# aosokin/os2d

Measured on AMD Instinct MI355X. Metric: query-image-pairs/s (1280-px input, ResNet50, N-class), higher is better.
Workload: dtype fftx3 (as fft; the per-bin complex GEMM on the fp16 MFMA with spectra split into fp16 hi+lo, 3 MFMAs per product, fp32 accumulate)

## Files before the change

### include/os2d_hip.h

```cpp
#ifndef OS2D_HIP_H
#define OS2D_HIP_H

#include <stddef.h>

#ifdef __cplusplus
extern "C" {
#endif

#define OS2D_ABI_VERSION 9

#define OS2D_PRECISION_F32 0
#define OS2D_PRECISION_F16X3 1
#define OS2D_PRECISION_F16X2 2

#define OS2D_PRECISION_FFT 3

#define OS2D_PRECISION_FFT32 5

#define OS2D_PRECISION_FFTX3 4

int os2d_abi_version(void);

const char* os2d_last_error(void);

size_t os2d_packed_conv_floats(int layer );
size_t os2d_packed_bias_floats(int layer );
int os2d_pack_conv(int layer, int P, const float* w, const float* b, const float* bn_weight, const float* bn_bias,
                   const float* bn_running_mean, const float* bn_running_var, float bn_eps, float* packed_w,
                   float* packed_b, void* stream);

int os2d_class_prepare(const float* src, int C, int h, int w, int normalize, float* q15, float* qp, void* stream);
size_t os2d_class_prepare_workspace_floats(int B, int C);
int os2d_class_prepare_batch(const float* const* srcs, const int* sizes, int B, int C, int normalize, float* q15,
                             float* qp, float* workspace, void* stream);

int os2d_head_workspace_bytes(int A, int B, int C, int H, int W, int P, size_t* bytes);
int os2d_head_workspace_bytes_ex(int A, int B, int C, int H, int W, int P, int precision, size_t* bytes);
int os2d_head_forward(const float* fm, const float* qp, const float* w1, const float* b1, const float* w2,
                      const float* b2, const float* w3, const float* b3, int A, int B, int C, int H, int W, int P,
                      int inverse, int stride, int rec_field, float* loc, float* cls, float* corners,
                      void* workspace, size_t workspace_bytes, void* stream);

size_t os2d_packed_conv_bytes(int layer, int precision);
int os2d_rnorm_exp(void);
int os2d_pack_conv_f16x3(int layer , int P, const float* w, const float* b, const float* bn_weight,
                         const float* bn_bias, const float* bn_running_mean, const float* bn_running_var, float bn_eps,
                         const int* weight_exp, const int* in_exp, const int* out_exp, void* packed_w, float* packed_b,
                         void* stream);

size_t os2d_class_split_bytes(int B, int C);
int os2d_class_split(const float* qp, void* qs, int B, int C, void* stream);

#define OS2D_STATUS_F16_RANGE 1
int os2d_head_forward_ex(const float* fm, const float* qp, const void* w1, const float* b1, const void* w2,
                         const float* b2, const void* w3, const float* b3, int A, int B, int C, int H, int W, int P,
                         int inverse, int stride, int rec_field, float* loc, float* cls, float* corners,
                         void* workspace, size_t workspace_bytes, void* stream, int precision, const void* qs,
                         void** stage_events, int* chunk_classes, int* status, const float* wspec, const float* twQ,
                         const float* twP);
int os2d_head_forward_ex2(const float* fm, const float* qp, const void* w1, const float* b1, const void* w2,
                          const float* b2, const void* w3, const float* b3, int A, int B, int C, int H, int W, int P,
                          int inverse, int stride, int rec_field, float* loc, float* cls, float* corners,
                          void* workspace, size_t workspace_bytes, void* stream, int precision, const void* qs,
                          void** stage_events, int* chunk_classes, int* status, const float* wspec, const float* twQ,
                          const float* twP, const void* wspec2);
void os2d_debug_set_dump(void* stream, int slot, void* dst, size_t bytes);
int os2d_prof_event_create(void** ev);
int os2d_prof_event_destroy(void* ev);
int os2d_prof_event_elapsed_ms(void* begin, void* end, float* ms);

int os2d_fm_sumsq(const float* fm, float* sumsq, int A, int C, int H, int W, void* stream);
size_t os2d_plane_floats(int H, int W);
int os2d_corr(const float* fm, const float* qp, const float* sumsq, float* corr, float* rnorm, int A, int B, int C,
              int H, int W, void* stream);
size_t os2d_corr_f16x3_workspace_bytes(int A, int C, int H, int W);
int os2d_corr_f16x3(const float* fm, const void* qs, float* corr, void* rshb, int A, int B, int C, int H, int W,
                    void* workspace, size_t workspace_bytes, void* stream);
size_t os2d_corr_f16x3_packed_workspace_bytes(int A, int B, int C, int H, int W);
int os2d_corr_f16x3_packed(const float* fm, const void* qs, float* corr, float* inv_norm, int A, int B, int C, int H, int W,
                           int form, void* workspace, size_t workspace_bytes, void* stream);
int os2d_corr_normalize(const float* corr, float* rnorm, int NB, int H, int W, void* stream);
int os2d_transform_conv(int layer, const float* in, const float* packed_w, const float* packed_b, float* out,
                        int NB, int P, int H, int W, void* stream);
size_t os2d_shb_bytes(int channels, int H, int W);
int os2d_corr_normalize_f16x3(const float* corr, void* rshb, int NB, int H, int W, void* stream);
int os2d_transform_conv_f16x3(int layer, const void* in, const void* packed_w, const float* packed_b, void* out, int NB,
                              int P, int H, int W, int terms, int* status, void* stream);
int os2d_alignment_grids(const float* params, int NB, int H, int W, int P, int inverse, float* theta, float* grids,
                         void* stream);
int os2d_sample_decode(const float* corr, const float* params, int NB, int H, int W, int P, int inverse, int stride,
                       int rec_field, float* loc, float* cls, float* corners, void* stream);

int os2d_decode_boxes(const float* loc, int NB, int H, int W, int stride, int rec_field, float img_w, float img_h,
                      float* boxes, void* stream);

int os2d_nms_workspace_bytes(int NC, int N, size_t* bytes);
int os2d_nms(const float* boxes, const int* counts, int NC, int N, float iou_threshold, unsigned char* keep,
             int* num_keep, void* workspace, size_t workspace_bytes, void* stream);

int os2d_detect_level_supported(int H, int W);
int os2d_detect_level(const float* loc, const float* cls, int B, int H, int W, int stride, int rec_field, float img_w,
                      float img_h, float scale_x, float scale_y, float score_threshold, float iou_threshold,
                      float* out_boxes, float* out_scores, int* out_index, int* out_count, void* stream);

#define OS2D_BOX_OP_SCALE 1
#define OS2D_BOX_OP_HFLIP 2
#define OS2D_BOX_OP_VFLIP 3
#define OS2D_BOX_OP_SHIFT 4
#define OS2D_BOX_MAX_OPS 6
#define OS2D_BOX_MAX_DEFAULT_OPS 12
int os2d_detect_level_ops(const float* loc, const float* cls, int B, int H, int W, int stride, int rec_field, float img_w,
                          float img_h, int op_count, const int* op_kinds, const float* op_args, float score_threshold,
                          float iou_threshold, float* out_boxes, float* out_scores, int* out_index, int* out_count,
                          void* stream);

size_t os2d_spectral_weight_bytes(int C, int Cout, int nbins);
int os2d_fft_sizes(int H, int W, int* P, int* Q, int* nbins);
int os2d_fft_tiles(int H, int W, int* tiles_y, int* tiles_x, int* tile_h, int* tile_w);
int os2d_fft_forward(const float* corr, const float* inv_norm, float* X, const float* twQ, const float* twP, int NB, int C,
                     int H, int W, void* stream);
int os2d_fft_inverse(const float* Y, const float* packed_b, void* out, const float* twQ, const float* twP, int NB, int Cout,
                     int H, int W, int* status, void* stream);
#define OS2D_SPECTRA_ROWS 0
#define OS2D_SPECTRA_QUADS 1
int os2d_fft_inverse_ex(const float* Y, const float* packed_b, void* out, const float* twQ, const float* twP, int NB, int Cout,
                        int H, int W, int* status, int layout, void* stream);
int os2d_spectral_gemm(const float* wspec, const float* X, float* Y, int NB, int C, int Cout, int nbins, void* stream);
size_t os2d_spectral_weight16_bytes(int C, int nbins);
int os2d_spectral_weights_build(const double* wfold, const double* twP64, const double* twQ64, int C, int Cout, int P, int Q,
                                int nbins, int split, void* out, void* workspace, void* stream);
float os2d_spectral_xscale(int H, int W);
int os2d_spectral_gemm_f16(const void* w16, const float* X, float* Y, int NB, int C, int Cout, int nbins, float xscale,
                           void* stream);

int os2d_dft_sizes(int H, int W, int* P, int* Q, int* nbins, int* tiles);
int os2d_dft_channel_stride(int C);
size_t os2d_dft_matrices_bytes(int P, int Q);
int os2d_dft_matrices_build(const double* twP64, const double* twQ64, int P, int Q, void* out, void* stream);
int os2d_dft_forward(const float* corr, const float* inv_norm, float* X, const void* matrices, int NB, int C, int H, int W,
                     void* stream);
int os2d_dft_inverse(const float* Y, const float* packed_b, void* out, const void* matrices, int NB, int Cout, int H, int W,
                     int* status, void* stream);
int os2d_dft_inverse_planes(const float* Y, const float* packed_b, float* out, const void* matrices, int NB, int Cout, int H, int W,
                            int* status, void* stream);
int os2d_spectral_weights_build_dft(const double* wfold, const double* twP64, const double* twQ64, int C, int Cout, int P, int Q,
                                    int nbins, void* out, void* workspace, void* stream);
int os2d_spectral_gemm_f16_quads(const void* w16, const float* X, float* Y, int NB, int C, int Cout, int nbins, float xscale,
                                 void* stream);
float os2d_dft_xscale(int H, int W);

#define OS2D_PYRAMID_MAX_LEVELS 16
int os2d_detect_pyramid_supported(int L, int N, int nms_max_batch);
int os2d_detect_pyramid_workspace_bytes(int B, int N, int passes, size_t* bytes);
int os2d_detect_pyramid(const float* const* loc, const float* const* cls, const float* const* corners, int B, int L,
                        const int* hw, int stride, int rec_field, const float* img_wh, const float* scale_xy,
                        float score_threshold, float iou_threshold, int nms_max_batch, int passes, float* out_boxes,
                        float* out_scores, int* out_index, float* out_default, float* out_corners, int* out_count,
                        int* unfinished, void* workspace, size_t workspace_bytes, void* stream);
int os2d_detect_pyramid_merged(const float* const* loc, const float* const* cls, const float* const* corners, int B, int L,
                               const int* hw, int stride, int rec_field, const float* img_wh, const float* scale_xy,
                               float score_threshold, float iou_threshold, int nms_max_batch, int passes, int G, int V,
                               const int* slot_rows, float* out_boxes, float* out_scores, int* out_index, float* out_default,
                               float* out_corners, int* out_count, int* unfinished, void* workspace, size_t workspace_bytes,
                               void* stream);

int os2d_detect_pyramid_ops(const float* const* loc, const float* const* cls, const float* const* corners, int B, int L,
                            const int* hw, int stride, int rec_field, const float* img_wh, const int* op_counts,
                            const int* op_kinds, const float* op_args, const int* default_op_counts,
                            const int* default_op_kinds, const float* default_op_args, float score_threshold, float iou_threshold,
                            int nms_max_batch, int passes, int G, int V, const int* slot_rows, float* out_boxes,
                            float* out_scores, int* out_index, float* out_default, float* out_corners, int* out_count,
                            int* unfinished, void* workspace, size_t workspace_bytes, void* stream);

#ifdef __cplusplus
}
#endif
#endif
```

### os2d_amd/_lib.py

```python
import ctypes

from . import build
from ._native import NativeLibrary, Os2dLibraryError, ptr, host_ptr, current_stream

ABI_VERSION = 9

_c_float_p = ctypes.c_void_p
_vp = ctypes.c_void_p
_i = ctypes.c_int
_f = ctypes.c_float
_sz = ctypes.c_size_t

SIGNATURES = {
    "os2d_abi_version": (_i, []),
    "os2d_last_error": (ctypes.c_char_p, []),
    "os2d_packed_conv_floats": (_sz, [_i]),
    "os2d_packed_bias_floats": (_sz, [_i]),
    "os2d_pack_conv": (_i, [_i, _i, _vp, _vp, _vp, _vp, _vp, _vp, _f, _vp, _vp, _vp]),
    "os2d_class_prepare": (_i, [_vp, _i, _i, _i, _i, _vp, _vp, _vp]),
    "os2d_head_workspace_bytes": (_i, [_i, _i, _i, _i, _i, _i, ctypes.POINTER(_sz)]),
    "os2d_head_forward": (_i, [_vp] * 8 + [_i] * 9 + [_vp, _vp, _vp, _vp, _sz, _vp]),
    "os2d_packed_conv_bytes": (_sz, [_i, _i]),
    "os2d_pack_conv_f16x3": (_i, [_i, _i, _vp, _vp, _vp, _vp, _vp, _vp, _f, _vp, _vp, _vp, _vp, _vp, _vp]),
    "os2d_rnorm_exp": (_i, []),
    "os2d_class_prepare_batch": (_i, [_vp, _vp, _i, _i, _i, _vp, _vp, _vp, _vp]),
    "os2d_class_prepare_workspace_floats": (_sz, [_i, _i]),
    "os2d_shb_bytes": (_sz, [_i, _i, _i]),
    "os2d_corr_normalize_f16x3": (_i, [_vp, _vp, _i, _i, _i, _vp]),
    "os2d_transform_conv_f16x3": (_i, [_i, _vp, _vp, _vp, _vp, _i, _i, _i, _i, _i, _vp, _vp]),
    "os2d_alignment_grids": (_i, [_vp, _i, _i, _i, _i, _i, _vp, _vp, _vp]),
    "os2d_spectral_weight_bytes": (_sz, [_i, _i, _i]),
    "os2d_spectral_gemm": (_i, [_vp, _vp, _vp, _i, _i, _i, _i, _vp]),
    "os2d_spectral_weight16_bytes": (_sz, [_i, _i]),
    "os2d_spectral_xscale": (_f, [_i, _i]),
    "os2d_spectral_weights_build": (_i, [_vp, _vp, _vp, _i, _i, _i, _i, _i, _i, _vp, _vp, _vp]),
    "os2d_spectral_gemm_f16": (_i, [_vp, _vp, _vp, _i, _i, _i, _i, _f, _vp]),
    "os2d_debug_set_dump": (None, [_vp, _i, _vp, _sz]),
    "os2d_fft_sizes": (_i, [_i, _i, ctypes.POINTER(_i), ctypes.POINTER(_i), ctypes.POINTER(_i)]),
    "os2d_fft_tiles": (_i, [_i, _i, ctypes.POINTER(_i), ctypes.POINTER(_i), ctypes.POINTER(_i), ctypes.POINTER(_i)]),
    "os2d_fft_forward": (_i, [_vp, _vp, _vp, _vp, _vp, _i, _i, _i, _i, _vp]),
    "os2d_fft_inverse": (_i, [_vp, _vp, _vp, _vp, _vp, _i, _i, _i, _i, _vp, _vp]),
    "os2d_fft_inverse_ex": (_i, [_vp, _vp, _vp, _vp, _vp, _i, _i, _i, _i, _vp, _i, _vp]),
    "os2d_dft_sizes": (_i, [_i, _i, ctypes.POINTER(_i), ctypes.POINTER(_i), ctypes.POINTER(_i), ctypes.POINTER(_i)]),
    "os2d_dft_channel_stride": (_i, [_i]),
    "os2d_dft_matrices_bytes": (_sz, [_i, _i]),
    "os2d_dft_matrices_build": (_i, [_vp, _vp, _i, _i, _vp, _vp]),
    "os2d_dft_forward": (_i, [_vp, _vp, _vp, _vp, _i, _i, _i, _i, _vp]),
    "os2d_dft_inverse": (_i, [_vp, _vp, _vp, _vp, _i, _i, _i, _i, _vp, _vp]),
    "os2d_spectral_weights_build_dft": (_i, [_vp, _vp, _vp, _i, _i, _i, _i, _i, _vp, _vp, _vp]),
    "os2d_spectral_gemm_f16_quads": (_i, [_vp, _vp, _vp, _i, _i, _i, _i, _f, _vp]),
    "os2d_dft_xscale": (_f, [_i, _i]),
    "os2d_class_split": (_i, [_vp, _vp, _i, _i, _vp]),
    "os2d_class_split_bytes": (_sz, [_i, _i]),
    "os2d_head_forward_ex": (_i, [_vp] * 8 + [_i] * 9 + [_vp, _vp, _vp, _vp, _sz, _vp, _i, _vp,
                                  ctypes.POINTER(_vp), ctypes.POINTER(_i), _vp, _vp, _vp, _vp]),
    "os2d_head_forward_ex2": (_i, [_vp] * 8 + [_i] * 9 + [_vp, _vp, _vp, _vp, _sz, _vp, _i, _vp,
                                   ctypes.POINTER(_vp), ctypes.POINTER(_i), _vp, _vp, _vp, _vp, _vp]),
    "os2d_dft_inverse_planes": (_i, [_vp, _vp, _vp, _vp, _i, _i, _i, _i, _vp, _vp]),
    "os2d_head_workspace_bytes_ex": (_i, [_i, _i, _i, _i, _i, _i, _i, ctypes.POINTER(_sz)]),
    "os2d_prof_event_create": (_i, [ctypes.POINTER(_vp)]),
    "os2d_prof_event_destroy": (_i, [_vp]),
    "os2d_prof_event_elapsed_ms": (_i, [_vp, _vp, ctypes.POINTER(_f)]),
    "os2d_fm_sumsq": (_i, [_vp, _vp, _i, _i, _i, _i, _vp]),
    "os2d_plane_floats": (_sz, [_i, _i]),
    "os2d_corr": (_i, [_vp, _vp, _vp, _vp, _vp, _i, _i, _i, _i, _i, _vp]),
    "os2d_corr_normalize": (_i, [_vp, _vp, _i, _i, _i, _vp]),
    "os2d_corr_f16x3_workspace_bytes": (_sz, [_i, _i, _i, _i]),
    "os2d_corr_f16x3": (_i, [_vp, _vp, _vp, _vp, _i, _i, _i, _i, _i, _vp, _sz, _vp]),
    "os2d_corr_f16x3_packed_workspace_bytes": (_sz, [_i, _i, _i, _i, _i]),
    "os2d_corr_f16x3_packed": (_i, [_vp, _vp, _vp, _vp, _i, _i, _i, _i, _i, _i, _vp, _sz, _vp]),
    "os2d_transform_conv": (_i, [_i, _vp, _vp, _vp, _vp, _i, _i, _i, _i, _vp]),
    "os2d_sample_decode": (_i, [_vp, _vp, _i, _i, _i, _i, _i, _i, _i, _vp, _vp, _vp, _vp]),
    "os2d_decode_boxes": (_i, [_vp, _i, _i, _i, _i, _i, _f, _f, _vp, _vp]),
    "os2d_nms_workspace_bytes": (_i, [_i, _i, ctypes.POINTER(_sz)]),
    "os2d_nms": (_i, [_vp, _vp, _i, _i, _f, _vp, _vp, _vp, _sz, _vp]),
    "os2d_detect_level_supported": (_i, [_i, _i]),
    "os2d_detect_level": (_i, [_vp, _vp] + [_i] * 5 + [_f] * 6 + [_vp] * 5),
    "os2d_detect_level_ops": (_i, [_vp, _vp] + [_i] * 5 + [_f, _f, _i, _vp, _vp, _f, _f] + [_vp] * 5),
    "os2d_detect_pyramid_supported": (_i, [_i, _i, _i]),
    "os2d_detect_pyramid_workspace_bytes": (_i, [_i, _i, _i, ctypes.POINTER(_sz)]),
    "os2d_detect_pyramid": (_i, [_vp, _vp, _vp, _i, _i, _vp, _i, _i, _vp, _vp, _f, _f, _i, _i, _vp, _vp, _vp, _vp, _vp, _vp,
                                 _vp, _vp, _sz, _vp]),
    "os2d_detect_pyramid_merged": (_i, [_vp, _vp, _vp, _i, _i, _vp, _i, _i, _vp, _vp, _f, _f, _i, _i, _i, _i, _vp, _vp, _vp, _vp,
                                        _vp, _vp, _vp, _vp, _vp, _sz, _vp]),
    "os2d_detect_pyramid_ops": (_i, [_vp, _vp, _vp, _i, _i, _vp, _i, _i, _vp, _vp, _vp, _vp, _vp, _vp, _vp, _f, _f, _i, _i, _i, _i, _vp, _vp, _vp,
                                     _vp, _vp, _vp, _vp, _vp, _vp, _sz, _vp]),
}


LIBRARY = NativeLibrary(build.HIP, SIGNATURES, ABI_VERSION, "os2d_abi_version", "os2d_last_error", "the OS2D head", __name__)
lib_path, load, check, call = LIBRARY.lib_path, LIBRARY.load, LIBRARY.check, LIBRARY.call
```

### os2d_amd/csrc/abi.hip

```cpp
#include "../../include/os2d_hip.h"
#include "abi_sizes.h"
#include "detect_common.h"

namespace {
bool conv_shape(int layer, int P, Os2dLayer* s) {
  if (layer < 1 || layer > 3) return false;
  *s = os2d_layer(layer, P);
  return true;
}
bool bad_P(int P) { return P != 6 && P != 4; }

int corr_f16x3_prologue(const float* fm, void* workspace, const CorrWorkspace& w, int A, int C, int H, int W, hipStream_t st, void** fs) {
  float* sumsq = reinterpret_cast<float*>(static_cast<char*>(workspace) + w.sumsq);
  *fs = static_cast<char*>(workspace) + w.fs;
  const int rc = os2d_launch_fm_sumsq(fm, sumsq, A, C, H * W, st);
  return rc ? rc : os2d_launch_split_fm(fm, sumsq, *fs, A, C, H * W, nullptr, 0, Os2dRangeFlag{nullptr, 0}, st);
}
bool bn_all_or_none(const float* weight, const float* bias, const float* mean, const float* var) {
  return (weight && bias && mean && var) || !(weight || bias || mean || var);
}
bool bad_bins(int nbins) { return nbins < 8 || (nbins & 7); }
bool spectral_gemm_args_ok(const char* who, const char* hint, const void* w, const float* X, const float* Y, int NB, int C, int Cout, int nbins,
                           float xscale) {
  if (!w || !X || !Y || NB < 1 || C < 1 || Cout < 1 || Cout > 128 || bad_bins(nbins) || !(xscale > 0.f))
    return OS2D_REFUSE(false, "%s: bad arguments (NB=%d C=%d Cout=%d nbins=%d%s)", who, NB, C, Cout, nbins, hint);
  if (!aligned_to(16, w, X, Y)) return OS2D_REFUSE(false, "%s: buffers must be 16-byte aligned", who);
  return true;
}
bool spectra_build_args_ok(const char* who, const double* wfold, const double* twP64, const double* twQ64, const void* out,
                           const void* workspace, bool need_workspace, int C, int Cout, int nbins, const int* P) {
  if (!wfold || !twP64 || !twQ64 || !out || (need_workspace && !workspace) || C < 1 || Cout < 1 || Cout > 128 || bad_bins(nbins) || (P && (*P & 3)))
    return P ? OS2D_REFUSE(false, "%s: bad arguments (C=%d Cout=%d P=%d nbins=%d)", who, C, Cout, *P, nbins)
             : OS2D_REFUSE(false, "%s: bad arguments (C=%d Cout=%d nbins=%d)", who, C, Cout, nbins);
  if (!aligned_to(16, out) || !aligned_to(8, workspace)) return OS2D_REFUSE(false, "%s: out must be 16-byte, workspace 8-byte aligned", who);
  return true;
}
bool dft_inverse_args_ok(const float* Y, const float* packed_b, const void* out, const void* matrices, int NB, int Cout, int H, int W) {
  return Y && packed_b && out && matrices && NB >= 1 && (Cout == os2d_layer(1).cout || Cout == os2d_layer(2).cout) && H >= 1 && W >= 1;
}
}

extern "C" {

int os2d_abi_version(void) { return OS2D_ABI_VERSION; }
const char* os2d_last_error(void) { return os2d_error_text; }

size_t os2d_packed_conv_floats(int layer) {
  Os2dLayer s;
  if (!conv_shape(layer, 6, &s)) return 0;
  return (size_t)(s.planes() / 2) * s.ks * s.ks * 2 * s.rows;
}
size_t os2d_packed_bias_floats(int layer) {
  Os2dLayer s;
  if (!conv_shape(layer, 6, &s)) return 0;
  return (size_t)3 * s.rows;
}

int os2d_pack_conv(int layer, int P, const float* w, const float* b, const float* bn_weight, const float* bn_bias,
                   const float* bn_running_mean, const float* bn_running_var, float bn_eps, float* packed_w,
                   float* packed_b, void* stream) {
  Os2dLayer s;
  if (!conv_shape(layer, P, &s) || (layer == 3 && bad_P(P))) return OS2D_REFUSE(-1, "os2d_pack_conv: bad layer %d / P %d", layer, P);
  if (!w || !b || !packed_w || !packed_b) return OS2D_REFUSE(-1, "os2d_pack_conv: null pointer");
  if (!bn_all_or_none(bn_weight, bn_bias, bn_running_mean, bn_running_var))
    return OS2D_REFUSE(-1, "os2d_pack_conv: BatchNorm needs all four of weight/bias/running_mean/running_var");
  return os2d_launch_pack_conv(w, b, bn_weight, bn_bias, bn_running_mean, bn_running_var, bn_eps, s.cout, s.cin, s.ks,
                               s.rows, packed_w, packed_b, os2d_stream(stream));
}

int os2d_class_prepare(const float* src, int C, int h, int w, int normalize, float* q15, float* qp, void* stream) {
  if (!src || !q15 || !qp || C < 1 || h < 1 || w < 1) return OS2D_REFUSE(-1, "os2d_class_prepare: bad arguments (C=%d h=%d w=%d)", C, h, w);
  return os2d_launch_class_prepare(src, C, h, w, normalize, q15, qp, os2d_stream(stream));
}

size_t os2d_class_prepare_workspace_floats(int B, int C) {
  if (B < 1 || C < 1) return 0;
  return (size_t)os2d_class_prepare_partial_floats(B, C);
}

int os2d_class_prepare_batch(const float* const* srcs, const int* sizes, int B, int C, int normalize, float* q15,
                             float* qp, float* workspace, void* stream) {
  if (!srcs || !sizes || !q15 || !qp || !workspace || B < 1 || C < 1 || B > 65535)
    return OS2D_REFUSE(-1, "os2d_class_prepare_batch: bad arguments (B=%d C=%d; at most 65535 classes per call)", B, C);
  return os2d_launch_class_prepare_batch(srcs, sizes, B, C, normalize, q15, qp, workspace, os2d_stream(stream));
}

size_t os2d_plane_floats(int H, int W) { return (size_t)os2d_plane(H, W); }

size_t os2d_shb_bytes(int channels, int H, int W) {
  if (channels < 1 || H < 1 || W < 1) return 0;
  return shb_bytes(channels, H, W);
}

int os2d_fm_sumsq(const float* fm, float* sumsq, int A, int C, int H, int W, void* stream) {
  if (!fm || !sumsq || A < 1 || C < 1 || H < 1 || W < 1) return OS2D_REFUSE(-1, "os2d_fm_sumsq: bad arguments");
  return os2d_launch_fm_sumsq(fm, sumsq, A, C, H * W, os2d_stream(stream));
}

int os2d_corr(const float* fm, const float* qp, const float* sumsq, float* corr, float* rnorm, int A, int B, int C,
              int H, int W, void* stream) {
  if (!fm || !qp || !sumsq || !corr || !rnorm) return OS2D_REFUSE(-1, "os2d_corr: null pointer");
  if (!head_args_ok(A, B, C, H, W, 6)) return -1;
  int rc = os2d_launch_border_zero(rnorm, A * B * OS2D_KP, H, W, os2d_stream(stream));
  if (rc) return rc;
  return os2d_launch_corr(fm, qp, sumsq, corr, rnorm, nullptr, A, B, C, H, W, 0, os2d_stream(stream));
}

size_t os2d_corr_f16x3_workspace_bytes(int A, int C, int H, int W) {
  if (A < 1 || C < 1 || H < 1 || W < 1) return 0;
  return corr_workspace(A, 0, C, H, W).total;
}

int os2d_corr_f16x3(const float* fm, const void* qs, float* corr, void* rshb, int A, int B, int C, int H, int W,
                    void* workspace, size_t workspace_bytes, void* stream) {
  if (!fm || !qs || !corr || !rshb || !workspace) return OS2D_REFUSE(-1, "os2d_corr_f16x3: null pointer");
  if (!head_args_ok(A, B, C, H, W, 6)) return -1;
  const CorrWorkspace w = corr_workspace(A, 0, C, H, W);
  if (workspace_bytes < w.total || !aligned_to(256, workspace)) return OS2D_REFUSE(-2, "os2d_corr_f16x3: workspace too small or not 256-byte aligned");
  void* fs;
  int rc = corr_f16x3_prologue(fm, workspace, w, A, C, H, W, os2d_stream(stream), &fs);
  if (!rc) rc = os2d_launch_border_zero_shb(rshb, A * B, H, W, os2d_stream(stream));
  if (!rc) rc = os2d_launch_corr_f16x3(fs, qs, corr, rshb, nullptr, nullptr, 0, A, B, C, H, W, os2d_stream(stream));
  return rc;
}

size_t os2d_corr_f16x3_packed_workspace_bytes(int A, int B, int C, int H, int W) {
  if (A < 1 || B < 1 || C < 1 || H < 1 || W < 1) return 0;
  return corr_workspace(A, B, C, H, W).total;
}

int os2d_corr_f16x3_packed(const float* fm, const void* qs, float* corr, float* inv_norm, int A, int B, int C, int H, int W,
                           int form, void* workspace, size_t workspace_bytes, void* stream) {
  if (!fm || !qs || !corr || !inv_norm || !workspace) return OS2D_REFUSE(-1, "os2d_corr_f16x3_packed: null pointer");
  if (!head_args_ok(A, B, C, H, W, 6)) return -1;
  if (form < -1 || form > 7 || (form >= 0 && (form & 3) > 1))
    return OS2D_REFUSE(-1, "os2d_corr_f16x3_packed: form %d (0 padded | 1 packed | -1 the head's choice; + 4: no half tiles at the tail)", form);
  const CorrWorkspace w = corr_workspace(A, B, C, H, W);
  if (workspace_bytes < w.total || !aligned_to(256, workspace))
    return OS2D_REFUSE(-2, "os2d_corr_f16x3_packed: workspace too small or not 256-byte aligned");
  void *fs, *sumfx = static_cast<char*>(workspace) + w.sumfx;
  int rc = corr_f16x3_prologue(fm, workspace, w, A, C, H, W, os2d_stream(stream), &fs);
  const bool packed = form < 0 ? os2d_corr_f16x3_use_packed(A, B, H, W) != 0 : (form & 1) != 0;
  if (!rc && packed) rc = os2d_launch_corr_sums_clear(sumfx, A, B, H, W, os2d_stream(stream));
  if (!rc) rc = os2d_launch_corr_f16x3(fs, qs, corr, nullptr, inv_norm, packed ? sumfx : nullptr, (form >= 0 && (form & 4)) ? 2 : 0, A, B, C, H, W, os2d_stream(stream));
  return rc;
}

int os2d_corr_normalize(const float* corr, float* rnorm, int NB, int H, int W, void* stream) {
  if (!corr || !rnorm || NB < 1 || H < 1 || W < 1) return OS2D_REFUSE(-1, "os2d_corr_normalize: bad arguments");
  return os2d_launch_corr_normalize(corr, rnorm, NB, H, W, os2d_stream(stream));
}

int os2d_transform_conv(int layer, const float* in, const float* packed_w, const float* packed_b, float* out, int NB,
                        int P, int H, int W, void* stream) {
  if (!in || !packed_w || !packed_b || !out || NB < 1 || H < 1 || W < 1 || (layer == 3 && bad_P(P)))
    return OS2D_REFUSE(-1, "os2d_transform_conv: bad arguments (layer=%d NB=%d P=%d)", layer, NB, P);
  return os2d_launch_conv(layer, in, packed_w, packed_b, out, NB, P, H, W, os2d_stream(stream));
}

int os2d_sample_decode(const float* corr, const float* params, int NB, int H, int W, int P, int inverse, int stride,
                       int rec_field, float* loc, float* cls, float* corners, void* stream) {
  if (!corr || !params || !loc || !cls || !corners || NB < 1 || H < 1 || W < 1 || bad_P(P)) return OS2D_REFUSE(-1, "os2d_sample_decode: bad arguments");
  return os2d_launch_sample_decode(corr, params, NB, H, W, P, inverse, stride, rec_field, NB, NB, 0, loc, cls,
                                   corners, nullptr, 0, nullptr, os2d_stream(stream));
}

int os2d_decode_boxes(const float* loc, int NB, int H, int W, int stride, int rec_field, float img_w, float img_h,
                      float* boxes, void* stream) {
  if (!loc || !boxes || NB < 1 || H < 1 || W < 1) return OS2D_REFUSE(-1, "os2d_decode_boxes: bad arguments");
  return os2d_launch_decode_boxes(loc, NB, H, W, stride, rec_field, img_w, img_h, boxes, os2d_stream(stream));
}

int os2d_detect_level_supported(int H, int W) { return os2d_detect_level_lds_bytes(H, W) != 0 ? 1 : 0; }

int os2d_detect_level(const float* loc, const float* cls, int B, int H, int W, int stride, int rec_field, float img_w,
                      float img_h, float scale_x, float scale_y, float score_threshold, float iou_threshold,
                      float* out_boxes, float* out_scores, int* out_index, int* out_count, void* stream) {
  if (!loc || !cls || !out_boxes || !out_scores || !out_index || !out_count || B < 1 || H < 1 || W < 1 || stride < 1 || rec_field < 1)
    return OS2D_REFUSE(-1, "os2d_detect_level: bad arguments");
  return os2d_launch_detect_level(loc, cls, B, H, W, stride, rec_field, img_w, img_h, os2d_box_ops_scale<OS2D_BOX_MAX_OPS>(scale_x, scale_y),
                                  score_threshold, iou_threshold, out_boxes, out_scores, out_index, out_count, os2d_stream(stream));
}

int os2d_detect_level_ops(const float* loc, const float* cls, int B, int H, int W, int stride, int rec_field, float img_w,
                          float img_h, int op_count, const int* op_kinds, const float* op_args, float score_threshold,
                          float iou_threshold, float* out_boxes, float* out_scores, int* out_index, int* out_count,
                          void* stream) {
  if (!loc || !cls || !out_boxes || !out_scores || !out_index || !out_count || B < 1 || H < 1 || W < 1 || stride < 1 || rec_field < 1)
    return OS2D_REFUSE(-1, "os2d_detect_level_ops: bad arguments");
  Os2dBoxOps ops;
  if (!os2d_box_ops_from(op_kinds, op_args, op_count, &ops))
    return OS2D_REFUSE(-1, "os2d_detect_level_ops: bad transform chain (at most %d ops of kind 1..4)", OS2D_BOX_MAX_OPS);
  return os2d_launch_detect_level(loc, cls, B, H, W, stride, rec_field, img_w, img_h, ops, score_threshold, iou_threshold,
                                  out_boxes, out_scores, out_index, out_count, os2d_stream(stream));
}

int os2d_nms_workspace_bytes(int NC, int N, size_t* bytes) {
  if (!bytes || NC < 1 || N < 1) return OS2D_REFUSE(-1, "os2d_nms_workspace_bytes: bad arguments");
  *bytes = nms_workspace_bytes(NC, N);
  return 0;
}

int os2d_nms(const float* boxes, const int* counts, int NC, int N, float iou_threshold, unsigned char* keep,
             int* num_keep, void* workspace, size_t workspace_bytes, void* stream) {
  if (!boxes || !counts || !keep || !num_keep || !workspace || NC < 1 || N < 1) return OS2D_REFUSE(-1, "os2d_nms: bad arguments");
  if (!aligned_to(16, boxes, workspace)) return OS2D_REFUSE(-1, "os2d_nms: boxes and workspace must be 16-byte aligned");
  if (workspace_bytes < nms_workspace_bytes(NC, N)) return OS2D_REFUSE(-2, "os2d_nms: workspace too small");
  return os2d_launch_nms(boxes, counts, NC, N, iou_threshold, keep, num_keep, workspace, os2d_stream(stream));
}

size_t os2d_class_split_bytes(int B, int C) {
  if (B < 1 || C < 1) return 0;
  return (size_t)B * class_split_bytes(C);
}

int os2d_class_split(const float* qp, void* qs, int B, int C, void* stream) {
  if (!qp || !qs || B < 1 || C < 1) return OS2D_REFUSE(-1, "os2d_class_split: bad arguments");
  return os2d_launch_split_qp(qp, qs, B, C, os2d_stream(stream));
}

size_t os2d_packed_conv_bytes(int layer, int precision) {
  if (precision == OS2D_PRECISION_F32) return os2d_packed_conv_floats(layer) * sizeof(float);
  if (precision != OS2D_PRECISION_F16X3 && precision != OS2D_PRECISION_F16X2) return 0;
  Os2dLayer s;
  if (!conv_shape(layer, 6, &s)) return 0;
  return (size_t)s.groups * s.steps * 4 * s.rows * 16;
}

int os2d_pack_conv_f16x3(int layer, int P, const float* w, const float* b, const float* bn_weight, const float* bn_bias,
                         const float* bn_running_mean, const float* bn_running_var, float bn_eps, const int* weight_exp,
                         const int* in_exp, const int* out_exp, void* packed_w, float* packed_b, void* stream) {
  Os2dLayer s;
  if (!conv_shape(layer, P, &s) || !w || !b || !packed_w || !packed_b || !weight_exp || !in_exp || (layer != 3 && !out_exp) ||
      !bn_all_or_none(bn_weight, bn_bias, bn_running_mean, bn_running_var) || (layer == 3 && bad_P(P)))
    return OS2D_REFUSE(-1, "os2d_pack_conv_f16x3: bad arguments (layer %d, P %d)", layer, P);
  return os2d_launch_pack_conv_f16(w, b, bn_weight, bn_bias, bn_running_mean, bn_running_var, bn_eps, s.cout, s.cin, s.ks, s.rows, s.steps,
                                   weight_exp, in_exp, layer == 3 ? nullptr : out_exp, packed_w, packed_b, os2d_stream(stream));
}

int os2d_rnorm_exp(void) { return OS2D_RNORM_EXP; }

int os2d_corr_normalize_f16x3(const float* corr, void* rshb, int NB, int H, int W, void* stream) {
  if (!corr || !rshb || NB < 1 || H < 1 || W < 1) return OS2D_REFUSE(-1, "os2d_corr_normalize_f16x3: bad arguments");
  return os2d_launch_corr_normalize_shb(corr, rshb, NB, H, W, os2d_stream(stream));
}

int os2d_transform_conv_f16x3(int layer, const void* in, const void* packed_w, const float* packed_b, void* out, int NB,
                              int P, int H, int W, int terms, int* status, void* stream) {
  if (!in || !packed_w || !packed_b || !out || NB < 1 || H < 1 || W < 1 || layer < 1 || layer > 3 || (layer == 3 && bad_P(P)) ||
      (terms != 3 && !(terms == 2 && layer == 1)))
    return OS2D_REFUSE(-1, "os2d_transform_conv_f16x3: bad arguments (layer=%d NB=%d P=%d terms=%d)", layer, NB, P, terms);
  const int max_w = layer == 1 ? OS2D_MAX_W_DIRECT7 : OS2D_MAX_W;
  if (W > max_w) return OS2D_REFUSE(-1, "os2d_transform_conv_f16x3: feature map width %d > %d", W, max_w);
  return os2d_launch_conv_f16x3(layer, in, packed_w, packed_b, Os2dRangeFlag{status, OS2D_STATUS_F16_RANGE}, out, NB, P, H, W, terms, os2d_stream(stream));
}

int os2d_fft_sizes(int H, int W, int* P, int* Q, int* nbins) {
  if (!P || !Q || !nbins) return OS2D_REFUSE(-1, "os2d_fft_sizes: null output");
  if (!os2d_fft_plan(H, W, P, Q, nbins, nullptr)) return OS2D_REFUSE(-3, "os2d_fft_sizes: no transform plan for a %dx%d map", H, W);
  return 0;
}

int os2d_fft_tiles(int H, int W, int* tiles_y, int* tiles_x, int* tile_h, int* tile_w) {
  int t[6];
  if (!tiles_y || !tiles_x || !tile_h || !tile_w) return OS2D_REFUSE(-1, "os2d_fft_tiles: null output");
  if (!os2d_fft_plan(H, W, nullptr, nullptr, nullptr, t)) return OS2D_REFUSE(-3, "os2d_fft_tiles: no transform plan for a %dx%d map", H, W);
  *tiles_y = t[0];
  *tiles_x = t[1];
  *tile_h = t[2];
  *tile_w = t[3];
  return 0;
}

int os2d_fft_forward(const float* corr, const float* inv_norm, float* X, const float* twQ, const float* twP, int NB, int C,
                     int H, int W, void* stream) {
  if (!corr || !inv_norm || !X || !twQ || !twP || NB < 1 || C < 1 || H < 1 || W < 1) return OS2D_REFUSE(-1, "os2d_fft_forward: bad arguments");
  return os2d_launch_fft_forward(corr, inv_norm, X, twQ, twP, NB, C, H, W, os2d_stream(stream));
}

int os2d_fft_inverse_ex(const float* Y, const float* packed_b, void* out, const float* twQ, const float* twP, int NB, int Cout,
                        int H, int W, int* status, int layout, void* stream) {
  constexpr Os2dLayer L1 = os2d_layer(1);
  if (!Y || !packed_b || !out || !twQ || !twP || NB < 1 || Cout != L1.cout || H < 1 || W < 1 || (layout != OS2D_SPECTRA_ROWS && layout != OS2D_SPECTRA_QUADS))
    return OS2D_REFUSE(-1, "os2d_fft_inverse: bad arguments (Cout must be 128: the 7x7 layer)");
  int rc = os2d_launch_border_zero_shb_planes(out, NB * (Cout / 8) * 2, H, W, os2d_stream(stream));
  if (rc) return rc;
  return os2d_launch_fft_inverse(Y, packed_b, L1.rows, out, twQ, twP, NB, Cout, H, W, Os2dRangeFlag{status, OS2D_STATUS_F16_RANGE}, layout, 0, os2d_stream(stream));
}

int os2d_fft_inverse(const float* Y, const float* packed_b, void* out, const float* twQ, const float* twP, int NB, int Cout,
                     int H, int W, int* status, void* stream) {
  return os2d_fft_inverse_ex(Y, packed_b, out, twQ, twP, NB, Cout, H, W, status, OS2D_SPECTRA_ROWS, stream);
}

size_t os2d_spectral_weight_bytes(int C, int Cout, int nbins) {
  if (C < 1 || Cout < 1 || Cout > 128 || bad_bins(nbins)) return 0;
  return os2d_spectral_weight_floats(C, Cout, nbins) * sizeof(float);
}

int os2d_spectral_gemm(const float* wspec, const float* X, float* Y, int NB, int C, int Cout, int nbins, void* stream) {
  if (!spectral_gemm_args_ok("os2d_spectral_gemm", "; nbins must be a multiple of 8", wspec, X, Y, NB, C, Cout, nbins, 1.f)) return -1;
  return os2d_launch_spectral_gemm(wspec, X, Y, NB, C, Cout, nbins, os2d_stream(stream));
}

int os2d_spectral_weights_build(const double* wfold, const double* twP64, const double* twQ64, int C, int Cout, int P, int Q,
                                int nbins, int split, void* out, void* workspace, void* stream) {
  if (!spectra_build_args_ok("os2d_spectral_weights_build", wfold, twP64, twQ64, out, workspace, split != 0, C, Cout, nbins, nullptr)) return -1;
  return os2d_launch_spectra_pack(wfold, twP64, twQ64, C, Cout, P, Q, nbins, split, 0, out, workspace, os2d_stream(stream));
}

size_t os2d_spectral_weight16_bytes(int C, int nbins) {
  if (C < 1 || bad_bins(nbins)) return 0;
  return os2d_spectral_weight16_size(C, nbins);
}

float os2d_spectral_xscale(int H, int W) {
  int t[6];
  if (H < 1 || W < 1 || !os2d_fft_plan(H, W, nullptr, nullptr, nullptr, t)) return 0.f;
  return os2d_spectral_xscale_for(t[4], t[5]);
}

int os2d_spectral_gemm_f16(const void* w16, const float* X, float* Y, int NB, int C, int Cout, int nbins, float xscale,
                           void* stream) {
  if (!spectral_gemm_args_ok("os2d_spectral_gemm_f16", "; nbins must be a multiple of 8", w16, X, Y, NB, C, Cout, nbins, xscale)) return -1;
  return os2d_launch_spectral_gemm_f16(w16, X, Y, NB, C, Cout, nbins, xscale, 0, 0, os2d_stream(stream));
}

int os2d_dft_sizes(int H, int W, int* P, int* Q, int* nbins, int* tiles) {
  if (!P || !Q || !nbins) return OS2D_REFUSE(-1, "os2d_dft_sizes: null output");
  if (!os2d_dft_plan(H, W, P, Q, nbins, tiles)) return OS2D_REFUSE(-3, "os2d_dft_sizes: no transform plan for a %dx%d map", H, W);
  return 0;
}

int os2d_dft_channel_stride(int C) { return C == OS2D_K ? OS2D_XSPEC_CPAD : (C + 7) / 8 * 8; }

size_t os2d_dft_matrices_bytes(int P, int Q) {
  if (P < 4 || (P & 3) || Q < 2 || (Q & 1)) return 0;
  return os2d_dft_matrices_size(P, Q);
}

int os2d_dft_matrices_build(const double* twP64, const double* twQ64, int P, int Q, void* out, void* stream) {
  if (!twP64 || !twQ64 || !out || !aligned_to(16, out)) return OS2D_REFUSE(-1, "os2d_dft_matrices_build: bad arguments (out must be 16-byte aligned)");
  return os2d_launch_dft_matrices(twP64, twQ64, P, Q, out, os2d_stream(stream));
}

int os2d_dft_forward(const float* corr, const float* inv_norm, float* X, const void* matrices, int NB, int C, int H, int W,
                     void* stream) {
  if (!corr || !X || !matrices || NB < 1 || C < 1 || H < 1 || W < 1) return OS2D_REFUSE(-1, "os2d_dft_forward: bad arguments");
  return os2d_launch_dft_forward(corr, inv_norm, X, matrices, NB, C, os2d_dft_channel_stride(C), H, W, os2d_stream(stream));
}

int os2d_dft_inverse(const float* Y, const float* packed_b, void* out, const void* matrices, int NB, int Cout, int H, int W,
                     int* status, void* stream) {
  if (!dft_inverse_args_ok(Y, packed_b, out, matrices, NB, Cout, H, W))
    return OS2D_REFUSE(-1, "os2d_dft_inverse: bad arguments (Cout must be 128 or 64: the 7x7 layer / the 5x5 layer 128 -> 64)");
  return os2d_launch_dft_inverse(Y, packed_b, Cout, out, matrices, NB, Cout, H, W, Os2dRangeFlag{status, OS2D_STATUS_F16_RANGE},
                                 OS2D_DFT_OUT_SHB_BORDERS, os2d_stream(stream));
}

int os2d_dft_inverse_planes(const float* Y, const float* packed_b, float* out, const void* matrices, int NB, int Cout, int H, int W,
                            int* status, void* stream) {
  if (!dft_inverse_args_ok(Y, packed_b, out, matrices, NB, Cout, H, W)) return OS2D_REFUSE(-1, "os2d_dft_inverse_planes: bad arguments (Cout must be 128 or 64)");
  return os2d_launch_dft_inverse(Y, packed_b, Cout, out, matrices, NB, Cout, H, W, Os2dRangeFlag{status, OS2D_STATUS_F16_RANGE},
                                 OS2D_DFT_OUT_PLANES, os2d_stream(stream));
}

int os2d_spectral_weights_build_dft(const double* wfold, const double* twP64, const double* twQ64, int C, int Cout, int P, int Q,
                                    int nbins, void* out, void* workspace, void* stream) {
  if (!spectra_build_args_ok("os2d_spectral_weights_build_dft", wfold, twP64, twQ64, out, workspace, true, C, Cout, nbins, &P)) return -1;
  return os2d_launch_spectra_pack(wfold, twP64, twQ64, C, Cout, P, Q, nbins, 1, 1, out, workspace, os2d_stream(stream));
}

int os2d_spectral_gemm_f16_quads(const void* w16, const float* X, float* Y, int NB, int C, int Cout, int nbins, float xscale,
                                 void* stream) {
  if (!spectral_gemm_args_ok("os2d_spectral_gemm_f16_quads", "", w16, X, Y, NB, C, Cout, nbins, xscale)) return -1;
  return os2d_launch_spectral_gemm_f16(w16, X, Y, NB, C, Cout, nbins, xscale, 1, os2d_dft_channel_stride(C), os2d_stream(stream));
}

float os2d_dft_xscale(int H, int W) {
  int t[6];
  if (H < 1 || W < 1 || !os2d_dft_plan(H, W, nullptr, nullptr, nullptr, t)) return 0.f;
  return os2d_spectral_xscale_for(t[4], t[5]);
}

int os2d_alignment_grids(const float* params, int NB, int H, int W, int P, int inverse, float* theta, float* grids,
                         void* stream) {
  if (!params || (!theta && !grids) || NB < 1 || H < 1 || W < 1 || bad_P(P)) return OS2D_REFUSE(-1, "os2d_alignment_grids: bad arguments");
  return os2d_launch_alignment_grids(params, NB, H, W, P, inverse, theta, grids, os2d_stream(stream));
}

int os2d_prof_event_create(void** ev) {
  hipEvent_t e;
  hipError_t rc = hipEventCreate(&e);
  if (rc != hipSuccess || !ev) return OS2D_REFUSE(-4, "hipEventCreate: %s", hipGetErrorString(rc));
  *ev = e;
  return 0;
}
int os2d_prof_event_destroy(void* ev) { return hipEventDestroy(reinterpret_cast<hipEvent_t>(ev)) == hipSuccess ? 0 : -4; }
int os2d_prof_event_elapsed_ms(void* a, void* b, float* ms) {
  hipError_t rc = hipEventElapsedTime(ms, reinterpret_cast<hipEvent_t>(a), reinterpret_cast<hipEvent_t>(b));
  if (rc != hipSuccess) return OS2D_REFUSE(-4, "hipEventElapsedTime: %s", hipGetErrorString(rc));
  return 0;
}

}
```

### os2d_amd/csrc/head_call.hip

```cpp
#include "../../include/os2d_hip.h"
#include "abi_sizes.h"
#include <atomic>
#include <mutex>
#include <random>
#include <vector>

namespace {
constexpr Os2dLayer L1 = os2d_layer(1), L2 = os2d_layer(2);

enum Transform7 { T7_NONE, T7_FFT, T7_DFT };
struct HeadRoute {
  int precision;
  bool f16;
  Transform7 transform;
  bool conv2_freq;
  bool borders_in_inverse;
  bool fused_tail_allowed;
  int terms1;
  int layout;
  int bins, tiles[6], T;
  int xch;
};

struct Span {
  size_t at, bytes;
};
struct Carve {
  Span flags, sumsq, fs, corr, rpad, h1, h2, params, invn, sumfx, xspec, yspec;
  size_t total;
};
Carve carve(const HeadRoute& r, int A, int Bc, int C, int H, int W, int P) {
  const size_t HW = (size_t)H * W, NB = (size_t)A * Bc, F = sizeof(float);
  Carve c = {};
  auto take = [&](size_t bytes) {
    const Span s = {c.total, bytes};
    c.total = align_up(c.total + bytes, 256);
    return s;
  };
  c.flags = take(((size_t)A + 1) * F);
  c.sumsq = take((size_t)A * HW * F);
  c.fs = take(fm_split_bytes(A, C, HW));
  c.corr = take(NB * L1.cin * HW * F);
  c.rpad = take(r.bins > 0 ? 0 : NB * shb_bytes(L1.cin, H, W));
  c.h1 = take(NB * L1.cout * os2d_plane(H, W) * F);
  c.h2 = take(NB * L2.cout * os2d_plane(H, W) * F);
  c.params = take(NB * P * HW * F);
  if (r.bins > 0) {
    c.invn = take(NB * HW * F);
    c.sumfx = take(NB * HW * sizeof(unsigned long long));
    c.xspec = take(NB * r.T * r.xch * (size_t)r.bins * 2 * F);
    c.yspec = take(NB * r.T * L1.cout * (size_t)r.bins * 2 * F);
  }
  return c;
}

#ifdef OS2D_DIAG_DUMP
struct DumpEntry {
  void* stream;
  int slot;
  void* dst;
  size_t bytes;
};
std::vector<DumpEntry> g_dumps;
std::mutex g_dumps_mutex;
bool dumps_active() {
  std::lock_guard<std::mutex> lock(g_dumps_mutex);
  return !g_dumps.empty();
}
void dump_slot(void* stream, int slot, const void* src, size_t bytes) {
  std::lock_guard<std::mutex> lock(g_dumps_mutex);
  for (const DumpEntry& e : g_dumps)
    if (e.stream == stream && e.slot == slot && e.dst)
      (void)hipMemcpyAsync(e.dst, src, bytes < e.bytes ? bytes : e.bytes, hipMemcpyDeviceToDevice, static_cast<hipStream_t>(stream));
}
#else
inline bool dumps_active() { return false; }
inline void dump_slot(void*, int, const void*, size_t) {}
#endif

int next_epoch() {
  static std::atomic<unsigned> counter{[] {
    std::random_device rd;
    return (unsigned)rd() | 0x100u;
  }()};
  unsigned e;
  do e = counter.fetch_add(1u, std::memory_order_relaxed) + 1u;
  while (e < 2u);
  return (int)e;
}
struct HeadSwitches {
  bool conv2_freq, borders_in_inverse, fused_tail;
};
bool env_on(const char* name) {
  const char* e = getenv(name);
  return !(e && e[0] == '0');
}
const HeadSwitches& head_switches() {
  static const HeadSwitches s = {env_on("OS2D_CONV2_FREQ"), env_on("OS2D_BORDERS_IN_INVERSE"), env_on("OS2D_FUSED_TAIL")};
  return s;
}
bool precision_route(int precision, HeadRoute* r) {
  *r = HeadRoute{precision, false, T7_NONE, false, false, false, 3, OS2D_SPECTRA_ROWS, 0, {1, 1, 0, 0, 0, 0}, 1, L1.cin};
  switch (precision) {
    case OS2D_PRECISION_F32: return true;
    case OS2D_PRECISION_F16X3: r->f16 = true; return true;
    case OS2D_PRECISION_F16X2: r->f16 = true, r->terms1 = 2; return true;
    case OS2D_PRECISION_FFT32: r->transform = T7_FFT; return true;
    case OS2D_PRECISION_FFT: r->f16 = true, r->transform = T7_FFT; return true;
    case OS2D_PRECISION_FFTX3: r->f16 = true, r->transform = T7_DFT, r->layout = OS2D_SPECTRA_QUADS, r->xch = OS2D_XSPEC_CPAD; return true;
    default: return false;
  }
}
int head_route(const char* who, int precision, int H, int W, bool have_wspec2, bool launch, HeadRoute* r) {
  if (!precision_route(precision, r) && launch) return OS2D_REFUSE(-1, "%s: unknown precision %d", who, precision);
  if (r->transform == T7_NONE) {
    if (launch && W > OS2D_MAX_W_DIRECT7)
      return OS2D_REFUSE(-1, "feature map width %d > %d: the direct 7x7 kernels keep 3 halo rows of their input in LDS - wider maps need a "
                         "frequency-domain precision (fftx3 / fft / fft32), which tiles any width up to %d", W, OS2D_MAX_W_DIRECT7, OS2D_MAX_W);
  } else if (!(r->transform == T7_DFT ? os2d_dft_plan : os2d_fft_plan)(H, W, nullptr, nullptr, &r->bins, r->tiles)) {
    return OS2D_REFUSE(-3, "%s: no transform plan for a %dx%d map", who, H, W);
  }
  r->T = r->tiles[0] * r->tiles[1];
  r->conv2_freq = r->transform == T7_DFT && have_wspec2 && head_switches().conv2_freq;
  r->borders_in_inverse = r->transform == T7_DFT && head_switches().borders_in_inverse;
  r->fused_tail_allowed = r->f16 && head_switches().fused_tail && !dumps_active();
  return 0;
}
int head_workspace_bytes(const char* who, int A, int B, int C, int H, int W, int P, int precision, size_t* bytes) {
  if (!bytes) return OS2D_REFUSE(-1, "%s: null output", who);
  if (!head_args_ok(A, B, C, H, W, P)) return -1;
  HeadRoute r;
  if (const int rc = head_route(who, precision, H, W, false, false, &r)) return rc;
  *bytes = carve(r, A, B, C, H, W, P).total;
  return 0;
}
int largest_chunk(const HeadRoute& r, int A, int B, int C, int H, int W, int P, size_t workspace_bytes) {
  const size_t one = carve(r, A, 1, C, H, W, P).total;
  if (workspace_bytes < one) return 0;
  int Bc = B;
  while (Bc > 1 && carve(r, A, Bc, C, H, W, P).total > workspace_bytes) {
    const size_t per = carve(r, A, 2, C, H, W, P).total - one;
    int guess = per ? (int)((workspace_bytes - one) / per) + 1 : 1;
    if (guess >= Bc) guess = Bc - 1;
    if (guess < 1) guess = 1;
    Bc = guess;
  }
  return Bc;
}

struct HeadCall {
  const float *fm, *qp, *b1, *b2, *b3, *wspec, *twQ, *twP;
  const void *w1, *w2, *w3, *qs, *wspec2;
  int A, B, C, H, W, P, inverse, stride, rec_field;
  float *loc, *cls, *corners;
  int* status;
  void** events;
  hipStream_t st;
  Carve layout;
  float *sumsq, *corr, *rpad, *h1, *h2, *params, *invn, *xspec, *yspec;
  void *fsplit, *sumfx;
  int* flags;
  int epoch;
  Os2dRangeFlag per_image, whole_call;
};
void mark(const HeadCall& x, int b0, int idx) {
  if (x.events && b0 == 0 && x.events[idx]) (void)hipEventRecord(reinterpret_cast<hipEvent_t>(x.events[idx]), x.st);
}
void dump(const HeadCall& x, int b0, int slot, const void* src, size_t bytes) {
  if (b0 == 0 && dumps_active()) dump_slot(x.st, slot, src, bytes);
}

int stage_corr(const HeadRoute& r, const HeadCall& x, int b0, int bc) {
  const int NB = x.A * bc;
  int rc;
  if (!r.bins && (rc = r.f16 ? os2d_launch_border_zero_shb(x.rpad, NB, x.H, x.W, x.st) : os2d_launch_border_zero(x.rpad, NB * L1.planes(), x.H, x.W, x.st)))
    return rc;
  if (!r.f16) return os2d_launch_corr(x.fm, x.qp + (size_t)b0 * x.C * OS2D_QROWS, x.sumsq, x.corr, x.rpad, x.invn, x.A, bc, x.C, x.H, x.W, 0, x.st);
  const char* qsb = static_cast<const char*>(x.qs) + (size_t)b0 * class_split_bytes(x.C);
  return os2d_launch_corr_f16x3(x.fsplit, qsb, x.corr, x.rpad, x.invn, x.sumfx, 1, x.A, bc, x.C, x.H, x.W, x.st);
}
int stage_conv1(const HeadRoute& r, const HeadCall& x, int b0, int bc) {
  const int NB = x.A * bc, H = x.H, W = x.W;
  int rc;
  if (r.transform == T7_NONE)
    return r.f16 ? os2d_launch_conv_f16x3(1, x.rpad, x.w1, x.b1, x.whole_call, x.h1, NB, x.P, H, W, r.terms1, x.st)
                 : os2d_launch_conv(1, x.rpad, static_cast<const float*>(x.w1), x.b1, x.h1, NB, x.P, H, W, x.st);
  if (r.f16) {
    const int planes = (r.borders_in_inverse || r.conv2_freq) ? 0 : NB * L2.groups * 2;
    if ((planes || x.sumfx) && (rc = os2d_launch_border_zero_shb_planes_norms(x.h1, planes, H, W, x.sumfx, x.invn, (size_t)NB * H * W, x.st)))
      return rc;
  } else if ((rc = os2d_launch_border_zero(x.h1, NB * L1.cout, H, W, x.st))) {
    return rc;
  }
  mark(x, b0, 10);
  if (r.transform == T7_FFT) {
    if ((rc = os2d_launch_fft_forward(x.corr, x.invn, x.xspec, x.twQ, x.twP, NB, L1.cin, H, W, x.st))) return rc;
    mark(x, b0, 11);
    if ((rc = os2d_launch_spectral_gemm(x.wspec, x.xspec, x.yspec, NB * r.T, L1.cin, L1.cout, r.bins, x.st))) return rc;
    mark(x, b0, 12);
    return os2d_launch_fft_inverse(x.yspec, x.b1, L1.rows, x.h1, x.twQ, x.twP, NB, L1.cout, H, W, x.whole_call, r.layout, r.f16 ? 0 : 1, x.st);
  }
  if ((rc = os2d_launch_dft_forward(x.corr, x.invn, x.xspec, x.twQ, NB, L1.cin, r.xch, H, W, x.st))) return rc;
  mark(x, b0, 11);
  if ((rc = os2d_launch_spectral_gemm_f16(x.wspec, x.xspec, x.yspec, NB * r.T, L1.cin, L1.cout, r.bins, os2d_spectral_xscale_for(r.tiles[4], r.tiles[5]), 1, r.xch, x.st)))
    return rc;
  mark(x, b0, 12);
  return os2d_launch_dft_inverse(x.yspec, x.b1, L1.rows, x.h1, x.twQ, NB, L1.cout, H, W, x.whole_call,
                                 r.conv2_freq ? OS2D_DFT_OUT_PLANES : r.borders_in_inverse ? OS2D_DFT_OUT_SHB_BORDERS : OS2D_DFT_OUT_SHB, x.st);
}
int stage_conv2(const HeadRoute& r, const HeadCall& x, int b0, int bc) {
  const int NB = x.A * bc, H = x.H, W = x.W;
  const Carve& c = x.layout;
  int rc;
  dump(x, b0, 0, x.corr, c.corr.bytes);
  if (r.bins) {
    dump(x, b0, 1, x.invn, c.invn.bytes);
    dump(x, b0, 2, x.xspec, c.xspec.bytes / r.xch * L1.cin);
    dump(x, b0, 3, x.yspec, c.yspec.bytes);
  }
  dump(x, b0, 4, x.h1, r.conv2_freq ? c.h1.bytes / os2d_plane(H, W) * ((size_t)H * W) : c.h1.bytes);
  if (!r.conv2_freq)
    return r.f16 ? os2d_launch_conv_f16x3(2, x.h1, x.w2, x.b2, x.whole_call, x.h2, NB, x.P, H, W, 3, x.st)
                 : os2d_launch_conv(2, x.h1, static_cast<const float*>(x.w2), x.b2, x.h2, NB, x.P, H, W, x.st);
  if ((rc = os2d_launch_dft_forward(x.h1, nullptr, x.xspec, x.twQ, NB, L2.cin, L2.cin, H, W, x.st))) return rc;
  if ((rc = os2d_launch_spectral_gemm_f16(x.wspec2, x.xspec, x.yspec, NB * r.T, L2.cin, L2.cout, r.bins, os2d_spectral_xscale_for(r.tiles[4], r.tiles[5]), 1, L2.cin, x.st)))
    return rc;
  return os2d_launch_dft_inverse(x.yspec, x.b2, L2.rows, x.h2, x.twQ, NB, L2.cout, H, W, x.whole_call, OS2D_DFT_OUT_SHB_BORDERS, x.st);
}
int stage_conv3(const HeadRoute& r, const HeadCall& x, int b0, int bc) {
  const int NB = x.A * bc;
  dump(x, b0, 5, x.h2, x.layout.h2.bytes);
  if (r.fused_tail_allowed)
    return os2d_launch_conv3_sample_decode(x.h2, x.w3, x.b3, x.corr, NB, x.H, x.W, x.P, x.inverse, x.stride, x.rec_field, bc, x.B, b0, x.loc, x.cls,
                                           x.corners, x.flags, x.epoch, x.status, x.st);
  return r.f16 ? os2d_launch_conv_f16x3(3, x.h2, x.w3, x.b3, x.whole_call, x.params, NB, x.P, x.H, x.W, 3, x.st)
               : os2d_launch_conv(3, x.h2, static_cast<const float*>(x.w3), x.b3, x.params, NB, x.P, x.H, x.W, x.st);
}
int stage_sample(const HeadRoute& r, const HeadCall& x, int b0, int bc) {
  const int NB = x.A * bc;
  if (r.fused_tail_allowed) return 0;
  dump(x, b0, 6, x.params, x.layout.params.bytes);
  return os2d_launch_sample_decode(x.corr, x.params, NB, x.H, x.W, x.P, x.inverse, x.stride, x.rec_field, bc, x.B, b0, x.loc, x.cls, x.corners,
                                   x.flags, x.epoch, x.status, x.st);
}
}

void os2d_debug_set_dump(void* stream, int slot, void* dst, size_t bytes) {
#ifdef OS2D_DIAG_DUMP
  std::lock_guard<std::mutex> lock(g_dumps_mutex);
  for (size_t i = 0; i < g_dumps.size(); ++i)
    if (g_dumps[i].stream == stream && g_dumps[i].slot == slot) {
      if (dst) {
        g_dumps[i].dst = dst;
        g_dumps[i].bytes = bytes;
      } else {
        g_dumps.erase(g_dumps.begin() + i);
      }
      return;
    }
  if (dst) g_dumps.push_back(DumpEntry{stream, slot, dst, bytes});
#else
  (void)stream, (void)slot, (void)dst, (void)bytes;
  os2d_set_error("os2d_debug_set_dump: this library was built without -DOS2D_DIAG_DUMP (diagnostic builds only)");
#endif
}

extern "C" {

int os2d_head_workspace_bytes(int A, int B, int C, int H, int W, int P, size_t* bytes) {
  return head_workspace_bytes("os2d_head_workspace_bytes", A, B, C, H, W, P, OS2D_PRECISION_F32, bytes);
}

int os2d_head_workspace_bytes_ex(int A, int B, int C, int H, int W, int P, int precision, size_t* bytes) {
  return head_workspace_bytes("os2d_head_workspace_bytes_ex", A, B, C, H, W, P, precision, bytes);
}

int os2d_head_forward_ex2(const float* fm, const float* qp, const void* w1, const float* b1, const void* w2,
                          const float* b2, const void* w3, const float* b3, int A, int B, int C, int H, int W, int P,
                          int inverse, int stride, int rec_field, float* loc, float* cls, float* corners,
                          void* workspace, size_t workspace_bytes, void* stream, int precision, const void* qs,
                          void** stage_events, int* chunk_classes, int* status, const float* wspec, const float* twQ,
                          const float* twP, const void* wspec2) {
  if (!fm || !qp || !w1 || !b1 || !w2 || !b2 || !w3 || !b3 || !loc || !cls || !corners || !workspace) return OS2D_REFUSE(-1, "os2d_head_forward: null pointer");
  HeadRoute route;
  precision_route(precision, &route);
  if (route.transform != T7_NONE && (!wspec || !twQ || (route.transform != T7_DFT && !twP)))
    return OS2D_REFUSE(-1, "os2d_head_forward: the frequency-domain modes need the weight spectra and the transform tables "
                       "(fft / fft32: twQ, twP; fftx3: the matrices of os2d_dft_matrices_build as twQ)");
  int rc = head_route("os2d_head_forward", precision, H, W, wspec2 != nullptr, true, &route);
  if (rc) return rc;
  if (route.f16 && !qs) return OS2D_REFUSE(-1, "os2d_head_forward: precision f16x3 / f16x2 needs the split class operand (os2d_class_split)");
  if (!head_args_ok(A, B, C, H, W, P)) return -1;
  if (stride < 1 || rec_field < 1) return OS2D_REFUSE(-1, "os2d_head_forward: bad stride/rec_field %d/%d", stride, rec_field);
  if (!aligned_to(256, workspace)) return OS2D_REFUSE(-1, "os2d_head_forward: workspace must be 256-byte aligned");
  const int Bc = largest_chunk(route, A, B, C, H, W, P, workspace_bytes);
  if (!Bc)
    return OS2D_REFUSE(-2, "os2d_head_forward: workspace too small (%zu B, need >= %zu B for one class)", workspace_bytes,
                       carve(route, A, 1, C, H, W, P).total);
  if (chunk_classes) *chunk_classes = Bc;
  HeadCall x = {fm, qp, b1, b2, b3, wspec, twQ, twP, w1, w2, w3, qs, wspec2, A, B, C, H, W, P, inverse, stride, rec_field, loc, cls, corners,
                status, stage_events, os2d_stream(stream), carve(route, A, Bc, C, H, W, P)};
  const Carve& c = x.layout;
  char* ws = static_cast<char*>(workspace);
  auto floats = [&](const Span& s) { return reinterpret_cast<float*>(ws + s.at); };
  x.sumsq = floats(c.sumsq);
  x.fsplit = ws + c.fs.at;
  x.corr = floats(c.corr);
  x.rpad = route.bins ? nullptr : floats(c.rpad);
  x.h1 = floats(c.h1);
  x.h2 = floats(c.h2);
  x.params = floats(c.params);
  x.invn = route.bins ? floats(c.invn) : nullptr;
  x.xspec = route.bins ? floats(c.xspec) : nullptr;
  x.yspec = route.bins ? floats(c.yspec) : nullptr;
  x.sumfx = (route.bins && route.f16 && os2d_corr_f16x3_use_packed(A, Bc, H, W)) ? ws + c.sumfx.at : nullptr;
  x.flags = route.f16 ? reinterpret_cast<int*>(ws + c.flags.at) : nullptr;
  x.epoch = next_epoch();
  x.per_image = {x.flags, x.epoch};
  x.whole_call = {route.f16 ? x.flags + A : nullptr, x.epoch};

  if ((rc = os2d_launch_fm_sumsq(fm, x.sumsq, A, C, H * W, x.st))) return rc;
  if (route.f16 && (rc = os2d_launch_split_fm(fm, x.sumsq, x.fsplit, A, C, H * W, x.sumfx, x.sumfx ? (size_t)A * Bc * H * W : 0, x.per_image, x.st)))
    return rc;
  for (int b0 = 0; b0 < B; b0 += Bc) {
    const int bc = (B - b0 < Bc) ? (B - b0) : Bc;
    mark(x, b0, 0);
    if ((rc = stage_corr(route, x, b0, bc))) return rc;
    mark(x, b0, 1);
    mark(x, b0, 2);
    if ((rc = stage_conv1(route, x, b0, bc))) return rc;
    mark(x, b0, 3);
    mark(x, b0, 4);
    if ((rc = stage_conv2(route, x, b0, bc))) return rc;
    mark(x, b0, 5);
    mark(x, b0, 6);
    if ((rc = stage_conv3(route, x, b0, bc))) return rc;
    mark(x, b0, 7);
    mark(x, b0, 8);
    if ((rc = stage_sample(route, x, b0, bc))) return rc;
    mark(x, b0, 9);
  }
  return 0;
}

int os2d_head_forward_ex(const float* fm, const float* qp, const void* w1, const float* b1, const void* w2,
                         const float* b2, const void* w3, const float* b3, int A, int B, int C, int H, int W, int P,
                         int inverse, int stride, int rec_field, float* loc, float* cls, float* corners,
                         void* workspace, size_t workspace_bytes, void* stream, int precision, const void* qs,
                         void** stage_events, int* chunk_classes, int* status, const float* wspec, const float* twQ,
                         const float* twP) {
  return os2d_head_forward_ex2(fm, qp, w1, b1, w2, b2, w3, b3, A, B, C, H, W, P, inverse, stride, rec_field, loc, cls, corners, workspace,
                               workspace_bytes, stream, precision, qs, stage_events, chunk_classes, status, wspec, twQ, twP, nullptr);
}

int os2d_head_forward(const float* fm, const float* qp, const float* w1, const float* b1, const float* w2,
                      const float* b2, const float* w3, const float* b3, int A, int B, int C, int H, int W, int P,
                      int inverse, int stride, int rec_field, float* loc, float* cls, float* corners, void* workspace,
                      size_t workspace_bytes, void* stream) {
  return os2d_head_forward_ex(fm, qp, w1, b1, w2, b2, w3, b3, A, B, C, H, W, P, inverse, stride, rec_field, loc, cls,
                              corners, workspace, workspace_bytes, stream, OS2D_PRECISION_F32, nullptr, nullptr, nullptr,
                              nullptr, nullptr, nullptr, nullptr);
}

}
```

### os2d_amd/csrc/os2d_common.h

```cpp
#pragma once
#include <hip/hip_runtime.h>
#include <stdint.h>

#include "../csrc_shared/abi_common.h"

#define OS2D_PAD 3
#define OS2D_T 15
#define OS2D_K 225
#define OS2D_KP 226
#define OS2D_QROWS 256
#define OS2D_MAX_W_DIRECT7 209
#define OS2D_MAX_W_LINEAR5 316
#define OS2D_MAX_W 3600
#define OS2D_MAX_H 2784
#define OS2D_XSPEC_CPAD 232
#define OS2D_G 29
#define OS2D_RNORM_EXP 12
#define OS2D_STATUS_F16_RANGE 1

struct Os2dLayer {
  int cout, cin, ks;
  int rows;
  int groups;
  int steps;
  constexpr int planes() const { return (cin + 1) / 2 * 2; }
};
constexpr Os2dLayer os2d_layer(int layer , int P = 6) {
  return layer == 1 ? Os2dLayer{128, OS2D_K, 7, 128, OS2D_G, 25} : layer == 2 ? Os2dLayer{64, 128, 5, 64, 16, 14} : Os2dLayer{P, 64, 5, 32, 8, 14};
}
static_assert(os2d_layer(1).planes() == OS2D_KP && os2d_layer(1).groups == (OS2D_K + 7) / 8 && os2d_layer(2).groups * 8 == os2d_layer(2).cin &&
                  os2d_layer(3).groups * 8 == os2d_layer(3).cin && os2d_layer(2).cin == os2d_layer(1).cout && os2d_layer(3).cin == os2d_layer(2).cout,
              "layer table");

struct Os2dRangeFlag {
  int* word;
  int value;
};
#ifdef __HIPCC__
__device__ __forceinline__ void os2d_raise(Os2dRangeFlag f) {
  __hip_atomic_store(f.word, f.value, __ATOMIC_RELAXED, __HIP_MEMORY_SCOPE_SYSTEM);
}
#endif

typedef float f32x16 __attribute__((ext_vector_type(16)));
typedef float f32x4 __attribute__((ext_vector_type(4)));

static inline __host__ __device__ int os2d_round_up(int x, int m) { return ((x + m - 1) / m) * m; }
static inline __host__ __device__ int os2d_ws(int W) { return W + OS2D_PAD; }
static inline __host__ __device__ int os2d_base(int W) { return os2d_round_up(OS2D_PAD * os2d_ws(W) + OS2D_PAD, 4); }
static inline __host__ __device__ int os2d_plane(int H, int W) {
  return os2d_round_up(os2d_base(W) + (H + OS2D_PAD) * os2d_ws(W) + OS2D_PAD, 64);
}
__device__ __forceinline__ void os2d_corr_norm_finalize_one(unsigned long long* __restrict__ sumfx, float* __restrict__ invn, size_t i) {
  const unsigned long long v = sumfx[i];
  sumfx[i] = 0ull;
  const float s = (v >> 62) ? __builtin_nanf("") : (float)((double)v * 5.6843418860808015e-14);
  invn[i] = 1.0f / (sqrtf(s) + 1e-6f);
}
template <class T>
__device__ __forceinline__ void os2d_stream_store(T* p, const T& v) {
  __builtin_nontemporal_store(v, p);
}
__device__ __forceinline__ unsigned os2d_split_lo_pair(float x0, float x1, unsigned hi) {
  unsigned lo;
  asm("v_fma_mixlo_f16 %0, %1, 1.0, -%3 op_sel_hi:[0,0,1]\n\t"
      "v_fma_mixhi_f16 %0, %2, 1.0, -%3 op_sel:[0,0,1] op_sel_hi:[0,0,1]"
      : "=&v"(lo)
      : "v"(x0), "v"(x1), "v"(hi));
  return lo;
}
__device__ __forceinline__ float os2d_relu(float v) { return v < 0.f ? 0.f : v; }
static inline __host__ __device__ bool os2d_interior(int n, int H, int W) {
  const int r = n - os2d_base(W);
  return r >= 0 && r < H * os2d_ws(W) && (r % os2d_ws(W)) < W;
}

int os2d_launch_fm_sumsq(const float* fm, float* sumsq, int A, int C, int HW, hipStream_t stream);
int os2d_launch_border_zero(float* rpad, int planes_total, int H, int W, hipStream_t stream);
int os2d_launch_corr_normalize(const float* corr, float* rpad, int NB, int H, int W, hipStream_t stream);
int os2d_launch_class_prepare(const float* src, int C, int h, int w, int normalize, float* q15, float* qp, hipStream_t stream);
int os2d_launch_pack_conv(const float* w, const float* b, const float* bn_w, const float* bn_b,
                          const float* bn_mean, const float* bn_var, float bn_eps, int Cout, int Cin, int KS,
                          int MT, float* wp, float* bp, hipStream_t stream);
int os2d_launch_border_zero_shb(void* rnorm, int NB, int H, int W, hipStream_t stream);
int os2d_launch_border_zero_shb_planes(void* buf, int planes, int H, int W, hipStream_t stream);
int os2d_launch_border_zero_shb_planes_norms(void* buf, int planes, int H, int W, void* sumfx, float* invn, size_t n, hipStream_t stream);
int os2d_launch_pack_conv_f16(const float* w, const float* b, const float* bn_w, const float* bn_b, const float* bn_mean,
                              const float* bn_var, float bn_eps, int Cout, int Cin, int KS, int MT, int steps_padded,
                              const int* wexp, const int* in_exp, const int* out_exp, void* wp, float* bp,
                              hipStream_t stream);
int os2d_class_prepare_partial_floats(int B, int C);
int os2d_launch_class_prepare_batch(const float* const* srcs, const int* sizes, int B, int C, int normalize, float* q15,
                                    float* qp, float* partial, hipStream_t stream);
int os2d_launch_corr_normalize_shb(const float* corr, void* rshb, int NB, int H, int W, hipStream_t stream);
int os2d_launch_corr(const float* fm, const float* qp, const float* sumsq, float* corr, void* rnorm ,
                     float* invn ,
                     int A, int B, int C, int H, int W, int shb, hipStream_t stream);
int os2d_launch_conv3_f16x3(const void* in, const void* wp, const float* bp, void* out, int NB, int P, int H, int W,
                            hipStream_t stream);
int os2d_launch_conv3_sample_decode(const void* in, const void* wp, const float* bp, const float* corr, int NB, int H, int W, int P,
                                    int inverse, int stride, int rec_field, int Bc, int Btot, int b0, float* loc, float* cls, float* corners,
                                    const int* flags, int epoch, int* host_status, hipStream_t stream);
int os2d_launch_conv_f16x3(int layer, const void* in, const void* wp, const float* bp, Os2dRangeFlag status, void* out, int NB,
                           int P, int H, int W, int terms, hipStream_t stream);
int os2d_launch_conv(int layer, const float* in, const float* wp, const float* bp, float* out,
                     int NB, int P, int H, int W, hipStream_t stream);
int os2d_launch_sample_decode(const float* corr, const float* params, int NB, int H, int W, int P, int inverse,
                              int stride, int rec_field, int Bc, int Btot, int b0, float* loc, float* cls,
                              float* corners, const int* flags , int epoch,
                              int* host_status , hipStream_t stream);
int os2d_launch_decode_boxes(const float* loc, int NB, int H, int W, int stride, int rec_field, float img_w,
                             float img_h, float* boxes, hipStream_t stream);
int os2d_launch_alignment_grids(const float* params, int NB, int H, int W, int P, int inverse, float* theta,
                                float* grids, hipStream_t stream);
int os2d_launch_nms(const float* boxes, const int* counts, int NC, int N, float thr, unsigned char* keep, int* num_keep,
                    void* workspace, hipStream_t stream);
int os2d_fft_plan(int H, int W, int* P, int* Q, int* nbins, int* tiles );
int os2d_launch_fft_forward(const float* corr, const float* inv, float* X, const float* twQ, const float* twP, int NB, int C,
                            int H, int W, hipStream_t stream);
int os2d_launch_fft_inverse(const float* Y, const float* bp, int MTP, void* out, const float* twQ, const float* twP, int NB,
                            int Cout, int H, int W, Os2dRangeFlag status, int layout ,
                            int out_fp32 ,
                            hipStream_t stream);
int os2d_launch_spectra_pack(const double* wfold, const double* twP64, const double* twQ64, int C, int Cout, int P, int Q,
                             int NBINS, int split, int u_fastest ,
                             void* out, void* workspace, hipStream_t stream);
size_t os2d_spectral_weight_floats(int C, int Cout, int NBINS);
int os2d_launch_spectral_gemm(const float* wspec, const float* X, float* Y, int NB, int C, int Cout, int NBINS,
                              hipStream_t stream);
size_t os2d_spectral_weight16_size(int C, int NBINS);
float os2d_spectral_xscale_for(int H, int W);
int os2d_launch_spectral_gemm_f16(const void* w16, const float* X, float* Y, int NB, int C, int Cout, int NBINS, float xscale,
                                  int x_quads , int Cpad,
                                  hipStream_t stream);
int os2d_dft_plan(int H, int W, int* P, int* Q, int* nbins, int* tiles );
size_t os2d_dft_matrices_size(int P, int Q);
int os2d_launch_dft_matrices(const double* twP64, const double* twQ64, int P, int Q, void* out, hipStream_t stream);
int os2d_launch_dft_forward(const float* corr, const float* inv, float* X, const void* matrices, int NB, int C, int Cpad, int H, int W,
                            hipStream_t stream);
enum { OS2D_DFT_OUT_SHB = 0, OS2D_DFT_OUT_SHB_BORDERS = 1, OS2D_DFT_OUT_PLANES = 2 };
int os2d_launch_dft_inverse(const float* Y, const float* bp, int MTP, void* out, const void* matrices, int NB, int Cout, int H, int W,
                            Os2dRangeFlag status, int form, hipStream_t stream);
int os2d_corr_groups(int C);
int os2d_launch_split_fm(const float* fm, const float* sumsq, void* fs, int A, int C, int HW, void* clear, size_t clear_words,
                         Os2dRangeFlag status, hipStream_t stream);
int os2d_launch_split_qp(const float* qp, void* qs, int B, int C, hipStream_t stream);
int os2d_launch_corr_f16x3(const void* fs, const void* qs, float* corr, void* rshb, float* invn, void* sumfx, int flags, int A,
                           int B, int C, int H, int W, hipStream_t stream);
int os2d_corr_f16x3_use_packed(int A, int B, int H, int W);
int os2d_launch_corr_sums_clear(void* sumfx, int A, int B, int H, int W, hipStream_t stream);
```

### os2d_amd/csrc/spectra_pack.hip

```cpp
#include "tile_common.h"

namespace {

constexpr int SP_THR = 256;
constexpr int SP_KS = 7, SP_TAPS = 49, SP_R = 3;

struct cd {
  double re, im;
};

__device__ __forceinline__ cd sp_value(const double (&w)[SP_TAPS], const cd* __restrict__ tP, const cd* __restrict__ tQ, int u,
                                       int v, int P, int Q) {
  cd ep[SP_KS], eq[SP_KS];
#pragma unroll
  for (int t = 0; t < SP_KS; ++t) {
    const int pt = (SP_R - t + P) % P, ps = (SP_R - t + Q) % Q;
    ep[t] = tP[(u * pt) % P];
    eq[t] = tQ[(v * ps) % Q];
  }
  cd k{0.0, 0.0};
#pragma unroll
  for (int s = 0; s < SP_KS; ++s) {
    double rr = 0.0, ri = 0.0;
#pragma unroll
    for (int t = 0; t < SP_KS; ++t) {
      rr = fma(w[t * SP_KS + s], ep[t].re, rr);
      ri = fma(w[t * SP_KS + s], ep[t].im, ri);
    }
    k.re = fma(rr, eq[s].re, fma(-ri, eq[s].im, k.re));
    k.im = fma(rr, eq[s].im, fma(ri, eq[s].re, k.im));
  }
  return k;
}

template <int MODE>
__global__ __launch_bounds__(SP_THR) void spectra_pack_kernel(const double* __restrict__ wfold,
                                                              const double* __restrict__ twP, const double* __restrict__ twQ,
                                                              int C, int Cout, int P, int Q, int NBINS, int bins_per_block,
                                                              unsigned long long* __restrict__ amax, void* __restrict__ out,
                                                              float* __restrict__ wscale, int ufast) {
  extern __shared__ __attribute__((aligned(16))) unsigned char smem[];
  cd* tP = reinterpret_cast<cd*>(smem);
  cd* tQ = tP + P;
  const int tid = threadIdx.x, lane = tid & 63, wv = tid >> 6;
  for (int i = tid; i < P; i += SP_THR) tP[i] = cd{twP[2 * i], twP[2 * i + 1]};
  for (int i = tid; i < Q; i += SP_THR) tQ[i] = cd{twQ[2 * i], twQ[2 * i + 1]};
  __syncthreads();
  const int V = Q / 2 + 1, KSTEPS = (C + 7) / 8;
  const int cu = blockIdx.x % (KSTEPS * 2), half = blockIdx.x / (KSTEPS * 2);
  const int c4 = MODE == 1 ? (lane & 3) : wv;
  const int ol = MODE == 1 ? wv * 16 + (lane >> 2) : lane;
  const int c = cu * 4 + c4, o = half * 64 + ol;
  const bool live = c < C && o < Cout;
  double w[SP_TAPS];
#pragma unroll
  for (int k = 0; k < SP_TAPS; ++k) w[k] = live ? wfold[((size_t)o * C + c) * SP_TAPS + k] : 0.0;
  const int bin0 = blockIdx.y * bins_per_block, bin1 = min(bin0 + bins_per_block, NBINS);
  if (MODE == 0) {
    double m = 0.0;
    for (int bin = bin0; bin < min(bin1, P * V); ++bin) {
      const int u = ufast ? bin % P : bin / V, v = ufast ? bin / P : bin - u * V;
      const cd k = sp_value(w, tP, tQ, u, v, P, Q);
      m = fmax(m, fmax(fabs(k.re), fabs(k.im)));
    }
    if (live) atomicMax(amax + o, (unsigned long long)__double_as_longlong(m));
    return;
  }
  double scale = 1.0;
  if (MODE == 1) {
    const double mx = o < Cout ? __longlong_as_double((long long)amax[o]) : 0.0;
    int e = mx > 0.0 ? (int)floor(log2(32768.0 / mx)) : 0;
    e = max(-100, min(100, e));
    scale = ldexp(1.0, e);
    if (blockIdx.x % (KSTEPS * 2) == 0 && blockIdx.y == 0 && c4 == 0 && o < 128) wscale[o] = (float)ldexp(1.0, -e);
  }
  for (int bin = bin0; bin < bin1; ++bin) {
    cd k{0.0, 0.0};
    if (bin < P * V) {
      const int u = ufast ? bin % P : bin / V, v = ufast ? bin / P : bin - u * V;
      k = sp_value(w, tP, tQ, u, v, P, Q);
    }
    const int g = bin >> 3, j = bin & 7;
    if (MODE == 1) {
      const double vr = k.re * scale, vi = k.im * scale;
      const _Float16 hr = (_Float16)vr, hi_ = (_Float16)vi;
      const _Float16 lr = (_Float16)(vr - (double)hr), li = (_Float16)(vi - (double)hi_);
      const unsigned hbits = (unsigned)__builtin_bit_cast(unsigned short, hr) | ((unsigned)__builtin_bit_cast(unsigned short, hi_) << 16);
      const unsigned lbits = (unsigned)__builtin_bit_cast(unsigned short, lr) | ((unsigned)__builtin_bit_cast(unsigned short, li) << 16);
      const int ks = cu >> 1, grp = cu & 1;
      const size_t unit = ((((((size_t)g * 2 + half) * KSTEPS + ks) * 8 + j) * 2 + grp) * 2) * 64 + ol;
      unsigned* dst = reinterpret_cast<unsigned*>(out) + unit * 4 + c4;
      dst[0] = hbits;
      dst[64 * 4] = lbits;
    } else {
      if (c < C) {
        float2* dst = reinterpret_cast<float2*>(out) + ((((size_t)g * 2 + half) * C + c) * 8 + j) * 64 + ol;
        *dst = make_float2((float)k.re, (float)k.im);
      }
    }
  }
}

}

int os2d_launch_spectra_pack(const double* wfold, const double* twP64, const double* twQ64, int C, int Cout, int P, int Q,
                             int NBINS, int split, int u_fastest, void* out, void* workspace, hipStream_t stream) {
  const int V = Q / 2 + 1, KSTEPS = (C + 7) / 8;
  if (P * V > NBINS || (NBINS & 7) || Cout > 128 || P < 1 || Q < 2 || (Q & 1)) {
    os2d_set_error("spectra_pack: bad sizes (P=%d Q=%d NBINS=%d Cout=%d)", P, Q, NBINS, Cout);
    return -3;
  }
  const size_t lds = (size_t)(P + Q) * sizeof(cd);
  const int nb_y = 8, per = os2d_round_up((NBINS + nb_y - 1) / nb_y, 8);
  dim3 grid(2 * KSTEPS * 2, (NBINS + per - 1) / per);
  if (split) {
    unsigned long long* amax = static_cast<unsigned long long*>(workspace);
    hipError_t e = hipMemsetAsync(amax, 0, 128 * sizeof(unsigned long long), stream);
    if (e != hipSuccess) {
      os2d_set_error("hipMemsetAsync: %s", hipGetErrorString(e));
      return -4;
    }
    hipLaunchKernelGGL(spectra_pack_kernel<0>, grid, dim3(SP_THR), lds, stream, wfold, twP64, twQ64, C, Cout, P, Q, NBINS, per, amax,
                       nullptr, nullptr, u_fastest);
    int rc = os2d_launched("spectra_pack (row maxima)");
    if (rc) return rc;
    float* wscale = reinterpret_cast<float*>(static_cast<char*>(out) + (size_t)(NBINS / 8) * 2 * KSTEPS * 8 * 256 * 16);
    hipLaunchKernelGGL(spectra_pack_kernel<1>, grid, dim3(SP_THR), lds, stream, wfold, twP64, twQ64, C, Cout, P, Q, NBINS, per, amax,
                       out, wscale, u_fastest);
    return os2d_launched("spectra_pack (split)");
  }
  hipLaunchKernelGGL(spectra_pack_kernel<2>, grid, dim3(SP_THR), lds, stream, wfold, twP64, twQ64, C, Cout, P, Q, NBINS, per, nullptr,
                     out, nullptr, u_fastest);
  return os2d_launched("spectra_pack (complex64)");
}
```

### os2d_amd/csrc/spectral_f16.hip

```cpp
#include "tile_common.h"

namespace {


constexpr int SH_THR = 512;
constexpr int SH_WB = 4;
constexpr int SH_BINS = 8;
constexpr int SH_OH = 64, SH_NB = 64;
constexpr int SH_KC = 8;
constexpr int SH_STAGE = SH_WB * 2 * 2 * 64;
constexpr int SH_WSTAGE = 2 * SH_STAGE;
constexpr int SH_WRING = 2;

#define SH_MM(x_, y_, acc_) __builtin_amdgcn_mfma_f32_32x32x16_f16(x_, y_, acc_, 0, 0, 0)
__device__ __forceinline__ void sh_lds_barrier() { asm volatile("s_waitcnt lgkmcnt(0)\n\ts_barrier" ::: "memory"); }

template <bool XQ, bool R64>
__device__ __forceinline__ void spectral_gemm_f16_body(const u32x4* w16,
                                                       const float* __restrict__ wscale,
                                                       const f32x2* __restrict__ X,
                                                       f32x2* __restrict__ Y,
                                                       int NB, int C, int Cpad, int Cout, int NBINS, float xscale, int nunits) {
  extern __shared__ __attribute__((aligned(16))) unsigned char smem[];
  constexpr int JB = R64 ? SH_WB / 2 : SH_WB;
  constexpr int WSTAGE = R64 ? SH_STAGE : SH_WSTAGE;
  constexpr int NWL = WSTAGE / SH_THR, NXL = SH_STAGE / SH_THR;
  u32x4* ldsW = reinterpret_cast<u32x4*>(smem);
  u32x4* ldsX = ldsW + SH_WRING * WSTAGE;
  const int tid = threadIdx.x, lane = tid & 63, l31 = lane & 31, hw = lane >> 5;
  const int wv = __builtin_amdgcn_readfirstlane(tid >> 6);
  const int lidx = os2d_xcd_logical(blockIdx.x, gridDim.x);
  if (lidx >= nunits) return;
  constexpr int NBH = SH_BINS / SH_WB;
  const int bh = lidx % NBH, lg = lidx / NBH;
  const int nbt = (NB + SH_NB - 1) / SH_NB;
  const int bt = lg % nbt, g = lg / nbt;
  const int nb0 = bt * SH_NB, bin0 = g * SH_BINS + bh * SH_WB;
  const int KS = (C + SH_KC - 1) / SH_KC;
  const int ot = R64 ? wv & 1 : wv & 3, pt = R64 ? (wv >> 1) & 1 : wv >> 2;
  const int wbp = R64 ? wv >> 2 : 0;
  const int wq = wv & 3, wh = wv >> 2;

  f32x16 yr[JB], yi[JB];
#pragma unroll
  for (int j = 0; j < JB; ++j)
#pragma unroll
    for (int r = 0; r < 16; ++r) {
      yr[j][r] = 0.f;
      yi[j][r] = 0.f;
    }

  const u32x4* wbase = w16 + ((size_t)(g * 2 + (R64 ? 0 : wh)) * KS) * (SH_BINS * 256) + bh * SH_STAGE;
#define SH_WRUN(K) (R64 ? wv * 2 + (K) : wq * 4 + (K))
#define SH_WPART (R64 ? 0 : wh * SH_STAGE)
  u32x4 wra[NWL], wrb[NWL];
#define SH_LOAD_W(S, wr)                                                                                            \
  {                                                                                                                 \
    const u32x4* src_ = wbase + (size_t)(S) * (SH_BINS * 256);                                                      \
    _Pragma("unroll") for (int k_ = 0; k_ < NWL; ++k_) wr[k_] = src_[SH_WRUN(k_) * 64 + lane];                      \
  }
#define SH_LOAD_W1(S, wr, K) wr[K] = (wbase + (size_t)(S) * (SH_BINS * 256))[SH_WRUN(K) * 64 + lane];
#define SH_STORE_W(S, wr)                                                                                           \
  {                                                                                                                 \
    _Pragma("unroll") for (int k_ = 0; k_ < NWL; ++k_)                                                              \
        ldsW[((S) % SH_WRING) * WSTAGE + SH_WPART + SH_WRUN(k_) * 64 + lane] = wr[k_];                             \
  }
  const int xn = XQ ? wv * 8 + (lane >> 3) : wq * 16 + (lane & 15);
  const int xj = XQ ? (lane & 1) : (lane >> 4) & 1, xg = XQ ? (lane >> 2) & 1 : lane >> 5;
  const int xwh = XQ ? (lane >> 1) & 1 : wh;
  const bool xn_ok = nb0 + xn < NB;
  const int nbl = min(SH_NB, NB - nb0);
  const size_t qblk = XQ ? (size_t)nb0 * (NBINS >> 2) + (size_t)(bin0 >> 2) * nbl : 0;
  const f32x2* xrow = XQ ? X + ((qblk + min(xn, nbl - 1)) * Cpad) * 4 + 2 * xj
                         : X + (size_t)min(nb0 + xn, NB - 1) * NBINS + bin0 + 2 * xj;
  const size_t xcs = XQ ? 4 : (size_t)NB * NBINS;
  u32x4 pfa[2], pfb[2];
#define SH_LOAD_X(S, pfx)                                                                                           \
  {                                                                                                                 \
    _Pragma("unroll") for (int i_ = 0; i_ < 2; ++i_) {                                                              \
      const int c_ = min((S)*SH_KC + xg * 4 + xwh * 2 + i_, C - 1);                                                 \
      pfx[i_] = *reinterpret_cast<const u32x4*>(xrow + (size_t)c_ * xcs);                                           \
    }                                                                                                               \
  }
#define SH_LOAD_X1(S, pfx, I)                                                                                       \
  {                                                                                                                 \
    const int c_ = min((S)*SH_KC + xg * 4 + xwh * 2 + (I), C - 1);                                                  \
    pfx[I] = *reinterpret_cast<const u32x4*>(xrow + (size_t)c_ * xcs);                                              \
  }
#define SH_STORE_X(S, pfx)                                                                                          \
  {                                                                                                                 \
    _Pragma("unroll") for (int b2_ = 0; b2_ < 2; ++b2_) {                                                           \
      f32x4 v4_;                                                                                                    \
      _Pragma("unroll") for (int i_ = 0; i_ < 2; ++i_) {                                                            \
        const bool ok_ = xn_ok && (S)*SH_KC + xg * 4 + xwh * 2 + i_ < C;                                            \
        _Pragma("unroll") for (int p_ = 0; p_ < 2; ++p_) {                                                          \
          const unsigned raw_ = pfx[i_][2 * b2_ + p_];    \
          v4_[2 * i_ + p_] = ok_ ? __uint_as_float(raw_) * xscale : 0.f;                                            \
        }                                                                                                           \
      }                                                                                                             \
      const half4 h_ = __builtin_convertvector(v4_, half4);                                                         \
      const u32x2 hp_ = __builtin_bit_cast(u32x2, h_);      \
      const u32x2 lp_ = {os2d_split_lo_pair(v4_[0], v4_[1], hp_[0]), os2d_split_lo_pair(v4_[2], v4_[3], hp_[1])};    \
      const half4 l_ = __builtin_bit_cast(half4, lp_);                                                              \
      char* dst_ = reinterpret_cast<char*>(ldsX + ((S)&1) * SH_STAGE + (((2 * xj + b2_) * 2 + xg) * 2) * 64 + xn) + xwh * 8; \
      *reinterpret_cast<half4*>(dst_) = h_;                    \
      *reinterpret_cast<half4*>(dst_ + 64 * 16) = l_;                                                               \
    }                                                                                                               \
  }
#define SH_REQUEST1(SN, WN, PN, R)  \
  if constexpr ((R) < NWL) {                                                                                        \
    SH_LOAD_W1(SN, WN, R)                                                                                           \
  } else if constexpr ((R) < NWL + NXL) {                                                                           \
    SH_LOAD_X1(SN, PN, (R)-NWL)                                                                                     \
  }
#define SH_REQUEST2(SN, WN, PN, R)                                                                                  \
  if constexpr ((R) < NWL + NXL) {                                                                                  \
    SH_REQUEST1(SN, WN, PN, R)                                                                                      \
    SH_REQUEST1(SN, WN, PN, (R) + 1)                                                                                \
    __builtin_amdgcn_sched_barrier(0);                                                                              \
  }
#define SH_REQUESTS_HOOK(SN, WN, PN, J)                                                                             \
  if ((J) == 0) {                                                                                                   \
    SH_REQUEST2(SN, WN, PN, 0)                                                                                      \
  } else if ((J) == 1) {                                                                                            \
    SH_REQUEST2(SN, WN, PN, 2)                                                                                      \
  } else if ((J) == 2) {                                                                                            \
    SH_REQUEST2(SN, WN, PN, 4)                                                                                      \
  }
#define SH_COMPUTE(S, SN, WN, PN)                                                                                         \
  {                                                                                                                 \
                                         \
    const u32x4* aB = ldsW + ((S) % SH_WRING) * WSTAGE + (R64 ? wbp * JB * 256 : (ot >> 1) * SH_STAGE) +            \
                      (hw * 2) * 64 + (ot & 1) * 32 + l31;                                                          \
    const u32x4* bB = ldsX + ((S)&1) * SH_STAGE + wbp * JB * 256 + (hw * 2) * 64 + pt * 32 + l31;                   \
    half8 bq[2][2];                                                                                                 \
    u32x4 kq[2][2];                                                                                                 \
    bq[0][0] = *reinterpret_cast<const half8*>(bB);                                                                 \
    bq[0][1] = *reinterpret_cast<const half8*>(bB + 64);                                                            \
    kq[0][0] = aB[0];                                                                                               \
    kq[0][1] = aB[64];                                                                                              \
    _Pragma("unroll") for (int j = 0; j < JB; ++j) {                                                                \
      if (j + 1 < JB) {                                                                                             \
        bq[(j + 1) & 1][0] = *reinterpret_cast<const half8*>(bB + (j + 1) * 256);                                   \
        bq[(j + 1) & 1][1] = *reinterpret_cast<const half8*>(bB + (j + 1) * 256 + 64);                              \
        kq[(j + 1) & 1][0] = aB[(j + 1) * 256];                                                                     \
        kq[(j + 1) & 1][1] = aB[(j + 1) * 256 + 64];                                                                \
      }                                                                                                             \
      __builtin_amdgcn_sched_barrier(0);                                                                            \
      const half8 bhf = bq[j & 1][0], blf = bq[j & 1][1];                                                           \
      const u32x4 kh = kq[j & 1][0], kl = kq[j & 1][1];                       \
      u32x4 rh, rl, ih, il;                                                                                         \
      _Pragma("unroll") for (int d = 0; d < 4; ++d) {                                                               \
        rh[d] = kh[d] ^ 0x80000000u;                                                                 \
        rl[d] = kl[d] ^ 0x80000000u;                                                                                \
        ih[d] = __builtin_amdgcn_alignbit(kh[d], kh[d], 16);                                          \
        il[d] = __builtin_amdgcn_alignbit(kl[d], kl[d], 16);                                                        \
      }                                                                                                             \
      const half8 arh = __builtin_bit_cast(half8, rh), arl = __builtin_bit_cast(half8, rl);                         \
      const half8 aih = __builtin_bit_cast(half8, ih), ail = __builtin_bit_cast(half8, il);                         \
       \
      yr[j] = SH_MM(bhf, arl, yr[j]);                                                                               \
      yr[j] = SH_MM(blf, arh, yr[j]);                                                                               \
      yr[j] = SH_MM(bhf, arh, yr[j]);                                                                               \
      yi[j] = SH_MM(bhf, ail, yi[j]);                                                                               \
      yi[j] = SH_MM(blf, aih, yi[j]);                                                                               \
      yi[j] = SH_MM(bhf, aih, yi[j]);                                                                               \
      __builtin_amdgcn_sched_barrier(0);                                                                            \
      SH_REQUESTS_HOOK(SN, WN, PN, j)                                                                               \
    }                                                                                                               \
  }
#define SH_STEP(S, WC, PC, WN, PN)                                                                                  \
  {                                                                                                                 \
    const int sn_ = min((S) + 2, KS - 1);                                                                           \
    SH_COMPUTE(S, sn_, WN, PN)                                                                                      \
    __builtin_amdgcn_sched_barrier(0);                                                                              \
    SH_STORE_W((S) + 1, WC)                                                                                         \
    SH_STORE_X((S) + 1, PC)                                                                                         \
    sh_lds_barrier();                                                                                               \
  }
  SH_LOAD_W(0, wrb)
  SH_LOAD_X(0, pfb)
  SH_LOAD_W(min(1, KS - 1), wra)
  SH_LOAD_X(min(1, KS - 1), pfa)
  SH_STORE_W(0, wrb)
  SH_STORE_X(0, pfb)
  sh_lds_barrier();
  int s = 0;
  for (; s + 1 < KS; s += 2) {
    SH_STEP(s, wra, pfa, wrb, pfb)
    SH_STEP(s + 1, wrb, pfb, wra, pfa)
  }
  if (s < KS) SH_STEP(s, wra, pfa, wrb, pfb)
#undef SH_STEP
#undef SH_REQUESTS_HOOK
#undef SH_REQUEST1
#undef SH_REQUEST2
#undef SH_WRUN
#undef SH_WPART
#undef SH_LOAD_W1
#undef SH_LOAD_X1
#undef SH_LOAD_W
#undef SH_STORE_W
#undef SH_COMPUTE
#undef SH_LOAD_X
#undef SH_STORE_X

  const float inv_x = 1.0f / xscale;
  const int o = ot * 32 + l31;
  if (o < Cout) {
    const float sc = wscale[o] * inv_x;
#pragma unroll
    for (int r = 0; r < 16; ++r) {
      const int nb = nb0 + pt * 32 + (r & 3) + 8 * (r >> 2) + 4 * hw;
      if (nb < NB) {
        float4* dst = XQ ? reinterpret_cast<float4*>(Y + ((qblk + (nb - nb0)) * Cout + o) * 4)
                         : reinterpret_cast<float4*>(Y + (((size_t)(bin0 >> 2) * NB + nb) * Cout + o) * 4);
        if constexpr (R64) {
          dst[wbp] = make_float4(yr[0][r] * sc, yi[0][r] * sc, yr[1][r] * sc, yi[1][r] * sc);
        } else {
          dst[0] = make_float4(yr[0][r] * sc, yi[0][r] * sc, yr[1][r] * sc, yi[1][r] * sc);
          dst[1] = make_float4(yr[2][r] * sc, yi[2][r] * sc, yr[3][r] * sc, yi[3][r] * sc);
        }
      }
    }
  }
}

template <bool XQ>
__global__ __launch_bounds__(SH_THR, 1) void spectral_gemm_f16_kernel(const u32x4* w16, const float* __restrict__ wscale,
                                                                      const f32x2* __restrict__ X, f32x2* __restrict__ Y, int NB, int C,
                                                                      int Cpad, int Cout, int NBINS, int rows64, float xscale,
                                                                      int nunits) {
  if (rows64)
    spectral_gemm_f16_body<XQ, true>(w16, wscale, X, Y, NB, C, Cpad, Cout, NBINS, xscale, nunits);
  else
    spectral_gemm_f16_body<XQ, false>(w16, wscale, X, Y, NB, C, Cpad, Cout, NBINS, xscale, nunits);
}

}

size_t os2d_spectral_weight16_size(int C, int NBINS) {
  const size_t KS = (size_t)(C + SH_KC - 1) / SH_KC;
  return (size_t)(NBINS / SH_BINS) * 2 * KS * SH_BINS * 256 * 16 + 128 * sizeof(float);
}

float os2d_spectral_xscale_for(int H, int W) {
  float s = 1.0f;
  while (s * 2.0f * (float)H * (float)W <= 65504.0f) s *= 2.0f;
  return s;
}

int os2d_launch_spectral_gemm_f16(const void* w16, const float* X, float* Y, int NB, int C, int Cout, int NBINS, float xscale,
                                  int x_quads, int Cpad, hipStream_t stream) {
  if (NBINS % SH_BINS || Cout > 2 * SH_OH) {
    os2d_set_error("spectral_gemm_f16: NBINS %d must be a multiple of %d and Cout %d <= %d", NBINS, SH_BINS, Cout, 2 * SH_OH);
    return -3;
  }
  if (x_quads && Cpad < C) {
    os2d_set_error("spectral_gemm_f16: channel stride %d < C %d", Cpad, C);
    return -1;
  }
  static const bool rows64_env = [] {
    const char* e = getenv("OS2D_GEMM_ROWS64");
    return !(e && e[0] == '0');
  }();
  const bool r64 = Cout <= SH_OH && rows64_env;
  const int G = NBINS / SH_BINS, nbt = (NB + SH_NB - 1) / SH_NB;
  const size_t KS = (size_t)(C + SH_KC - 1) / SH_KC;
  const float* wscale = reinterpret_cast<const float*>(static_cast<const char*>(w16) + (size_t)G * 2 * KS * SH_BINS * 256 * 16);
  const size_t lds = (size_t)(SH_WRING * (r64 ? SH_STAGE : SH_WSTAGE) + 2 * SH_STAGE) * 16;
  const long long units = (long long)G * nbt * (SH_BINS / SH_WB);
  unsigned grid;
  if (int rc = os2d_xcd_grid(units, "spectral_gemm_f16", &grid)) return rc;
  auto kern = x_quads ? spectral_gemm_f16_kernel<true> : spectral_gemm_f16_kernel<false>;
  if (int rc = os2d_set_dynamic_lds(kern, lds, "spectral_gemm_f16")) return rc;
  hipLaunchKernelGGL(kern, dim3(grid), dim3(SH_THR), lds, stream, static_cast<const u32x4*>(w16), wscale,
                     reinterpret_cast<const f32x2*>(X), reinterpret_cast<f32x2*>(Y), NB, C, Cpad, Cout, NBINS, (int)r64, xscale, (int)units);
  return os2d_launched("spectral_gemm_f16");
}
```

### os2d_amd/modeling/head.py

```python
import copy
import ctypes
import logging
import os
import weakref

import torch
import torch.nn as nn

from .. import _lib, _train_lib
from .._native import STREAM
from ..structures.feature_map import FeatureMapSize
from .box_coder import BoxGridGenerator
from . import head_train
from .device_buffers import (STATUS_SLOTS, _WORKSPACES, device_status_word, get_workspace, release_workspaces,
                             workspace_cap_bytes)
from .spectra import (_NET_IDS, _SpectraStore, _SpectraView, _StreamOrdered, _drop_spectra_of, build_dft_matrices,
                      build_weight_spectra, spectra_cache_cap_bytes, split_rows_f16, transform_sizes, twiddles64)

TEMPLATE = 15
QROWS = 256
MAX_W_DIRECT7 = 209
FFT_MIN_PAIRS = 7
PRECISIONS = {"f32": 0, "f16x3": 1, "f16x2": 2, "fft": 3, "fftx3": 4, "fft32": 5}
FFT_MODES = ("fft", "fftx3", "fft32")
FP32_MODES = ("f32", "fft32")
DEFAULT_PRECISION = "fftx3"
RANGE_PLAN_ROUTES = ("device", "torch")
DEFAULT_RANGE_PLAN = "device"


def resolve_range_plan_route(route=None):
    if route is None:
        route = os.environ.get("OS2D_RANGE_PLAN", DEFAULT_RANGE_PLAN)
    if route not in RANGE_PLAN_ROUTES:
        raise ValueError("range plan route must be one of {}, got {!r}".format(RANGE_PLAN_ROUTES, route))
    return route


def resolve_precision(precision=None):
    return _resolve(precision)[0]


def _resolve(precision=None):
    precision = precision or os.environ.get("OS2D_PRECISION", DEFAULT_PRECISION)
    pinned = isinstance(precision, str) and precision.endswith("!")
    name = precision[:-1] if pinned else precision
    if name not in PRECISIONS or (pinned and name not in FFT_MODES):
        raise ValueError("precision must be one of {} (\"fft!\" / \"fftx3!\" pin the frequency-domain route), got {!r}".format(
            sorted(PRECISIONS), precision))
    return name, pinned


def build_os2d_head_creator(do_simple_affine, is_cuda, use_inverse_geom_model, feature_map_stride,
                            feature_map_receptive_field):
    aligner = Os2dAlignment(do_simple_affine, is_cuda, use_inverse_geom_model)
    return Os2dHeadCreator(aligner, feature_map_stride, feature_map_receptive_field)


def _require_device_f32(t, name):
    if not isinstance(t, torch.Tensor):
        raise TypeError("{} must be a torch.Tensor".format(name))
    if not t.is_cuda:
        raise RuntimeError("{} is on {}: the OS2D head runs only on a HIP device (libos2d_hip.so); there is no "
                           "CPU fallback".format(name, t.device))
    if t.dtype != torch.float32:
        raise RuntimeError("{} must be float32, got {}".format(name, t.dtype))
    return t.contiguous()


class TransformationNet(nn.Module):

    range_plan_route = None

    def __init__(self, output_dim=6, use_cuda=True, normalization="batchnorm", kernel_sizes=[7, 5],
                 channels=[128, 64], input_feature_dim=15 * 15, num_groups=16):
        super(TransformationNet, self).__init__()
        if list(kernel_sizes) != [7, 5] or list(channels) != [128, 64] or input_feature_dim != 225:
            raise RuntimeError("the HIP TransformNet kernels are built for the OS2D architecture "
                               "(225 -> 128 k7 -> 64 k5 -> P k5)")
        if normalization.lower() != "batchnorm":
            raise RuntimeError("only 'batchnorm' TransformNet normalisation is supported (the reference "
                               "hard-codes it, head.py:72)")
        mods = []
        ch_in = input_feature_dim
        for ch_out, k in zip(channels, kernel_sizes):
            mods += [nn.Conv2d(ch_in, ch_out, kernel_size=k, padding=k // 2), nn.BatchNorm2d(ch_out),
                     nn.ReLU(inplace=True)]
            ch_in = ch_out
        self.conv = nn.Sequential(*mods)
        k = kernel_sizes[-1]
        self.linear = nn.Conv2d(ch_in, output_dim, kernel_size=(k, k), padding=k // 2)
        with torch.no_grad():
            self.linear.weight.zero_()
            self.linear.bias.zero_()
            if output_dim == 6:
                self.linear.bias[0] = 1
                self.linear.bias[4] = 1
            elif output_dim == 4:
                self.linear.bias[0] = 1
                self.linear.bias[2] = 1
        self.output_dim = output_dim
        self._packed_cache = {}
        self._new_net_id()
        if use_cuda:
            self.conv.cuda()
            self.linear.cuda()

    def _new_net_id(self):
        self._net_id = next(_NET_IDS)
        weakref.finalize(self, _drop_spectra_of, self._net_id)

    def __deepcopy__(self, memo):
        cls = self.__class__
        clone = cls.__new__(cls)
        memo[id(self)] = clone
        for k, v in self.__dict__.items():
            if k not in ("_net_id", "_packed_cache"):
                setattr(clone, k, copy.deepcopy(v, memo))
        clone._packed_cache = {}
        clone._new_net_id()
        return clone

    def __setstate__(self, state):
        super(TransformationNet, self).__setstate__(state)
        self._packed_cache = {}
        self._new_net_id()

    def freeze_bn(self):
        for layer in self.modules():
            if isinstance(layer, nn.BatchNorm2d):
                layer.eval()

    def live_batchnorm(self):
        return tuple(bool(self.training and bn.training) for bn in (self.conv[1], self.conv[4]))

    def check_ready(self, allow_live_batchnorm=False):
        dev = self.linear.weight.device
        if dev.type != "cuda":
            raise RuntimeError("TransformationNet parameters are on {}: move the model to the HIP device "
                               "(no CPU fallback)".format(dev))
        if self.training and any(isinstance(m, nn.BatchNorm2d) and m.training for m in self.modules()):
            if not allow_live_batchnorm:
                raise RuntimeError("TransformationNet is in training mode: the HIP path implements eval-mode "
                                   "BatchNorm (running statistics) only; call .eval()")
            for name, bn, live in zip(("conv.1", "conv.4"), (self.conv[1], self.conv[4]), self.live_batchnorm()):
                if live and bn.momentum is None:
                    raise ValueError("{}: momentum=None (a cumulative average) is not implemented for a training-mode BatchNorm".format(name))
                if live and not bn.track_running_stats:
                    raise ValueError("{}: track_running_stats=False is not implemented for a training-mode BatchNorm".format(name))
        return dev

    def packed_linear_f32(self):
        ts = (self.linear.weight, self.linear.bias)
        key = ("linear.f32",) + tuple((t.data_ptr(), t._version, str(t.device)) for t in ts)
        dev = self.linear.weight.device
        cached = self._packed_cache.get("linear.f32")
        if cached is not None and cached.key == key:
            return cached.get(dev)
        lib = _lib.load()
        with torch.cuda.device(dev):
            w = _require_device_f32(self.linear.weight.detach(), "conv weight")
            b = _require_device_f32(self.linear.bias.detach(), "conv bias")
            pw = torch.empty(lib.os2d_packed_conv_floats(3), dtype=torch.float32, device=dev)
            pb = torch.zeros(lib.os2d_packed_bias_floats(3), dtype=torch.float32, device=dev)
            _lib.call("os2d_pack_conv", 3, self.output_dim, w, b, None, None, None, None, 0.0, pw, pb, STREAM)
            result = (pw, pb)
            self._packed_cache["linear.f32"] = _StreamOrdered(key, result, dev)
        return result

    def _state_key(self):
        ts = list(self.parameters()) + list(self.buffers())
        return tuple((t.data_ptr(), t._version, str(t.device)) for t in ts)

    def _folded(self):
        out = []
        for conv, bn in ((self.conv[0], self.conv[1]), (self.conv[3], self.conv[4]), (self.linear, None)):
            w, b = conv.weight.detach().double(), conv.bias.detach().double()
            if bn is not None:
                s = bn.weight.detach().double() / torch.sqrt(bn.running_var.detach().double() + bn.eps)
                w = w * s.view(-1, 1, 1, 1)
                b = (b - bn.running_mean.detach().double()) * s + bn.bias.detach().double()
            out.append((w, b))
        return out

    def range_plan(self):
        (w1, b1), (w2, b2), (w3, b3) = self._folded()

        def floor_log2(x):
            ok = torch.isfinite(x) & (x > 0)
            e = torch.floor(torch.log2(torch.where(ok, x, torch.ones_like(x))))
            return torch.where(ok, e, torch.zeros_like(e)).clamp(-60, 60).to(torch.int32)

        def out_exp(bound):
            return floor_log2(32768.0 / bound.clamp_min(1e-300)) * (bound > 0).to(torch.int32)

        def weight_exp(w, in_exp):
            eff = w * torch.exp2(-in_exp.double()).view(1, -1, 1, 1)
            amax = eff.abs().amax(dim=(1, 2, 3))
            return floor_log2(16384.0 / amax.clamp_min(1e-300)) * (amax > 0).to(torch.int32)

        lib = _lib.load()
        bound1 = 7.0 * w1.flatten(1).norm(dim=1) + b1.abs()
        l1 = (w2.abs().sum(dim=(2, 3)) * bound1.view(1, -1)).sum(dim=1)
        l2 = 5.0 * bound1.norm() * w2.flatten(1).norm(dim=1)
        bound2 = torch.minimum(l1, l2) + b2.abs()
        e0 = torch.full((225,), lib.os2d_rnorm_exp(), dtype=torch.int32, device=w1.device)
        e1, e2 = out_exp(bound1), out_exp(bound2)
        return dict(in_exp=[e0, e1, e2], out_exp=[e1, e2, None], unit_exp=e1 - 15,
                    weight_exp=[weight_exp(w1, e0), weight_exp(w2, e1), weight_exp(w3, e2)], bounds=(bound1, bound2))

    _RANGE_PLAN_FIELDS = (128, 128, 128, 64, 64, 8)

    def _range_plan_buffers(self):
        key = ("range_plan",) + self._state_key()
        dev = self.check_ready()
        cached = self._packed_cache.get("range_plan")
        if cached is not None and cached.key == key:
            return cached.get(dev)
        lib = _train_lib.load()
        assert sum(self._RANGE_PLAN_FIELDS) == lib.os2d_train_range_plan_ints()
        with torch.cuda.device(dev):
            held, args = [], [self.output_dim]
            for conv, bn in ((self.conv[0], self.conv[1]), (self.conv[3], self.conv[4])):
                held += [_require_device_f32(t.detach(), "TransformNet parameter")
                         for t in (conv.weight, conv.bias, bn.weight, bn.bias, bn.running_mean, bn.running_var)]
                args += held[-6:] + [float(bn.eps)]
            held.append(_require_device_f32(self.linear.weight.detach(), "TransformNet parameter"))
            exps = torch.empty(lib.os2d_train_range_plan_ints(), dtype=torch.int32, device=dev)
            bounds = torch.empty(lib.os2d_train_range_plan_doubles(), dtype=torch.int64, device=dev)
            _train_lib.call("os2d_train_range_plan", *args, held[-1], exps, bounds, STREAM)
            result = (exps, bounds)
            self._packed_cache["range_plan"] = _StreamOrdered(key, result, dev)
        return result

    def _plan_views(self, exps, bounds):
        wexp1, e1, unit_exp, wexp2, e2, wexp3 = exps.split(self._RANGE_PLAN_FIELDS)
        e0 = torch.full((225,), _lib.load().os2d_rnorm_exp(), dtype=torch.int32, device=exps.device)
        return dict(in_exp=[e0, e1, e2], out_exp=[e1, e2, None], unit_exp=unit_exp, weight_exp=[wexp1, wexp2, wexp3[:self.output_dim]],
                    bounds=None if bounds is None else tuple(bounds.split((128, 64))))

    def range_plan_device(self):
        exps, bounds = self._range_plan_buffers()
        return self._plan_views(exps, bounds.view(torch.float64))

    def _f16x3_plan(self):
        if resolve_range_plan_route(self.range_plan_route) == "torch":
            return self.range_plan()
        return self._plan_views(self._range_plan_buffers()[0], None)

    def packed(self, precision=None):
        precision = resolve_precision(precision)
        if precision in ("f16x2", "fft", "fftx3"):
            precision = "f16x3"
        elif precision == "fft32":
            precision = "f32"
        key = (precision,) + self._state_key()
        dev = self.linear.weight.device
        cached = self._packed_cache.get(precision)
        if cached is not None and cached.key == key:
            return cached.get(dev)
        lib = _lib.load()
        self.check_ready()
        with torch.cuda.device(dev):
            cur = torch.cuda.current_stream(dev)
            out = []
            P = self.output_dim
            plan = self._f16x3_plan() if precision == "f16x3" else None
            if plan is not None:
                act = tuple(e.to(dev).contiguous() for e in (plan["in_exp"][0], plan["out_exp"][0], plan["out_exp"][1]))
                self._packed_cache["f16x3.act_exp"] = _StreamOrdered(key, act, dev)
            layers = ((1, self.conv[0], self.conv[1]), (2, self.conv[3], self.conv[4]), (3, self.linear, None))
            for layer, conv, bn in layers:
                w = _require_device_f32(conv.weight.detach(), "conv weight")
                b = _require_device_f32(conv.bias.detach(), "conv bias")
                pb = torch.zeros(lib.os2d_packed_bias_floats(layer), dtype=torch.float32, device=dev)
                if bn is not None:
                    bnp = [_require_device_f32(t.detach(), "bn") for t in (bn.weight, bn.bias, bn.running_mean, bn.running_var)]
                    eps = float(bn.eps)
                else:
                    bnp, eps = [None] * 4, 0.0
                if precision == "f16x3":
                    exps = [plan[k][layer - 1] for k in ("weight_exp", "in_exp", "out_exp")]
                    exps = [e.to(dev).contiguous() if e is not None else None for e in exps]
                    pw = torch.empty(lib.os2d_packed_conv_bytes(layer, PRECISIONS[precision]), dtype=torch.uint8, device=dev)
                    _lib.call("os2d_pack_conv_f16x3", layer, P, w, b, *bnp, eps, *exps, pw, pb, STREAM)
                    for e in exps:
                        if e is not None:
                            e.record_stream(cur)
                else:
                    pw = torch.empty(lib.os2d_packed_conv_floats(layer), dtype=torch.float32, device=dev)
                    _lib.call("os2d_pack_conv", layer, P, w, b, *bnp, eps, pw, pb, STREAM)
                out += [pw, pb]
            result = tuple(out)
            self._packed_cache[precision] = _StreamOrdered(key, result, dev)
        return result

    def activation_exponents(self):
        self.packed("f16x3")
        return self._packed_cache["f16x3.act_exp"].get(self.linear.weight.device)

    def _cached_spectra(self, H, W, split, slot_tag, build):
        dev = self.check_ready()
        plan = transform_sizes(int(H), int(W), bool(split))
        if plan is None:
            return None
        key, slot, store = self._state_key(), plan[:2] + (bool(split),) + slot_tag, _SpectraStore.of(dev)
        cached = store.get(self._net_id, slot, key)
        if cached is not None:
            return cached.get(dev)
        store.drop_stale(self._net_id, key)
        with torch.cuda.device(dev), torch.no_grad():
            result = build(*plan[:3], dev)
            store.put(self._net_id, slot, _StreamOrdered(key, result, dev))
        return result

    def spectra(self, H, W, split=False):
        def build(P, Q, nbins, dev):
            wspec = build_weight_spectra(self._folded()[0][0], 225, 128, P, Q, nbins, split, dev)
            if split:
                return wspec, build_dft_matrices(P, Q, dev), None, nbins
            return wspec, twiddles64(Q, dev).float(), twiddles64(P, dev).float(), nbins
        return self._cached_spectra(H, W, split, (), build)

    def spectra2(self, H, W):
        def build(P, Q, nbins, dev):
            _, (w2, _), _ = self._folded()
            unit_exp = self._f16x3_plan()["unit_exp"].to(w2.device).double()
            w2 = nn.functional.pad(w2 * torch.exp2(-unit_exp).view(1, -1, 1, 1), (1, 1, 1, 1))
            return build_weight_spectra(w2, 128, 64, P, Q, nbins, True, dev)
        return self._cached_spectra(H, W, True, ("conv2",), build)

    @property
    def _spectra_cache(self):
        dev = self.linear.weight.device
        return _SpectraView(_SpectraStore.of(dev), self._net_id) if dev.type == "cuda" else {}

    def forward(self, corr_maps, precision="f32"):
        corr_maps = _require_device_f32(corr_maps, "corr_maps")
        if corr_maps.dim() != 4 or corr_maps.size(1) != 225:
            raise RuntimeError("corr_maps must be [N,225,H,W], got {}".format(tuple(corr_maps.shape)))
        if torch.is_grad_enabled() and (corr_maps.requires_grad or any(p.requires_grad for p in self.parameters())) and self.training:
            raise RuntimeError("autograd through the HIP TransformNet is not implemented (training is out of scope)")
        precision = resolve_precision(precision)
        lib = _lib.load()
        N, _, H, W = corr_maps.shape
        dev = corr_maps.device
        P = self.output_dim
        w1, b1, w2, b2, w3, b3 = self.packed(precision)
        out = torch.empty(N, P, H, W, dtype=torch.float32, device=dev)
        with torch.cuda.device(dev):
            if precision in FP32_MODES:
                plane = lib.os2d_plane_floats(H, W)
                r = torch.empty(N * 226 * plane, dtype=torch.float32, device=dev)
                h1 = torch.empty(N * 128 * plane, dtype=torch.float32, device=dev)
                h2 = torch.empty(N * 64 * plane, dtype=torch.float32, device=dev)
                _lib.call("os2d_corr_normalize", corr_maps, r, N, H, W, STREAM)
                _lib.call("os2d_transform_conv", 1, r, w1, b1, h1, N, P, H, W, STREAM)
                _lib.call("os2d_transform_conv", 2, h1, w2, b2, h2, N, P, H, W, STREAM)
                _lib.call("os2d_transform_conv", 3, h2, w3, b3, out, N, P, H, W, STREAM)
            else:
                terms1 = 2 if precision == "f16x2" else 3
                r = torch.empty(N * lib.os2d_shb_bytes(225, H, W), dtype=torch.uint8, device=dev)
                h1 = torch.empty(N * lib.os2d_shb_bytes(128, H, W), dtype=torch.uint8, device=dev)
                h2 = torch.empty(N * lib.os2d_shb_bytes(64, H, W), dtype=torch.uint8, device=dev)
                status = torch.zeros(1, dtype=torch.int32, device=dev)
                _lib.call("os2d_corr_normalize_f16x3", corr_maps, r, N, H, W, STREAM)
                for layer, src, wp, bp, dst, terms in ((1, r, w1, b1, h1, terms1), (2, h1, w2, b2, h2, 3), (3, h2, w3, b3, out, 3)):
                    _lib.call("os2d_transform_conv_f16x3", layer, src, wp, bp, dst, N, P, H, W, terms, status, STREAM)
                self.last_status = status
        return out


class Os2dAlignment(nn.Module):

    def __init__(self, do_simple_affine, is_cuda, use_inverse_geom_model):
        super(Os2dAlignment, self).__init__()
        self.model_type = "affine" if not do_simple_affine else "simple_affine"
        self.use_inverse_geom_model = use_inverse_geom_model
        transform_net_output_dim = 6 if self.model_type == "affine" else 4
        self.out_grid_size = FeatureMapSize(w=TEMPLATE, h=TEMPLATE)
        self.reference_feature_map_size = FeatureMapSize(w=TEMPLATE, h=TEMPLATE)
        self.network_stride = FeatureMapSize(w=1, h=1)
        self.network_receptive_field = FeatureMapSize(w=TEMPLATE, h=TEMPLATE)
        self.input_feature_dim = TEMPLATE * TEMPLATE
        self.parameter_regressor = TransformationNet(output_dim=transform_net_output_dim, use_cuda=is_cuda,
                                                     normalization="batchnorm", kernel_sizes=[7, 5],
                                                     channels=[128, 64], input_feature_dim=self.input_feature_dim)

    @property
    def num_transform_params(self):
        return self.parameter_regressor.output_dim

    def prepare_transform_parameters_for_grid_sampler(self, transform_parameters):
        return self._grids(transform_parameters, want_theta=True, want_grids=False)[0]

    def _grids(self, params, want_theta, want_grids):
        params = _require_device_f32(params, "transform_parameters")
        N, P, H, W = params.shape
        assert P == self.num_transform_params, \
            "Tranformation parameter vector has to be of dimension {0}, have {1} instead".format(self.num_transform_params, P)
        dev = params.device
        theta = torch.empty(N * H * W, 2, 3, dtype=torch.float32, device=dev) if want_theta else None
        grids = torch.empty(N, H, W, TEMPLATE, TEMPLATE, 2, dtype=torch.float32, device=dev) if want_grids else None
        _lib.call("os2d_alignment_grids", params, N, H, W, P, 1 if self.use_inverse_geom_model else 0, theta, grids, STREAM)
        return theta, grids

    def forward(self, corr_maps, precision="f32"):
        assert corr_maps.size(1) == self.input_feature_dim, \
            "The dimension 1 of corr_maps={0} should be equal to self.input_feature_dim={1}".format(corr_maps.size(1), self.input_feature_dim)
        transform_parameters = self.parameter_regressor(corr_maps, precision=precision)
        return self._grids(transform_parameters, want_theta=False, want_grids=True)[1]


class Os2dHeadCreator(nn.Module):

    def __init__(self, aligner, feature_map_stride, feature_map_receptive_field):
        super(Os2dHeadCreator, self).__init__()
        self.aligner = aligner
        rec_field, stride = self.get_rec_field_and_stride_after_concat_nets(
            feature_map_receptive_field, feature_map_stride,
            self.aligner.network_receptive_field, self.aligner.network_stride)
        self.feature_map_stride = feature_map_stride
        self.feature_map_receptive_field = feature_map_receptive_field
        self.box_grid_generator_image_level = BoxGridGenerator(box_size=rec_field, box_stride=stride)
        self.box_grid_generator_feature_map_level = BoxGridGenerator(box_size=self.aligner.network_receptive_field,
                                                                     box_stride=self.aligner.network_stride)
        self.train_precision = None
        self.train_forward_precision = None
        self.deterministic = None

    @staticmethod
    def get_rec_field_and_stride_after_concat_nets(receptive_field_netA, stride_netA, receptive_field_netB, stride_netB):
        if isinstance(receptive_field_netA, FeatureMapSize):
            f = Os2dHeadCreator.get_rec_field_and_stride_after_concat_nets
            rw, sw = f(receptive_field_netA.w, stride_netA.w, receptive_field_netB.w, stride_netB.w)
            rh, sh = f(receptive_field_netA.h, stride_netA.h, receptive_field_netB.h, stride_netB.h)
            return FeatureMapSize(w=rw, h=rh), FeatureMapSize(w=sw, h=sh)
        return stride_netA * (receptive_field_netB - 1) + receptive_field_netA, stride_netA * stride_netB

    @staticmethod
    def resize_feature_maps_to_reference_size(ref_size, feature_maps):
        q15, _ = _prepare_class_maps(feature_maps, normalise=False)
        return q15

    def create_os2d_head(self, class_feature_maps):
        q15, qp = _prepare_class_maps(class_feature_maps, normalise=True)
        head = Os2dHead(q15, self.aligner, self.box_grid_generator_image_level,
                        self.box_grid_generator_feature_map_level, _prepared=qp,
                        _stride=self.feature_map_stride, _rec_field=self.feature_map_receptive_field)
        if isinstance(class_feature_maps, torch.Tensor):
            class_feature_maps = [m.unsqueeze(0) for m in class_feature_maps]
        head._raw_class_maps = list(class_feature_maps)
        head.train_precision = self.train_precision
        head.train_forward_precision = self.train_forward_precision
        head.deterministic = self.deterministic
        return head


def _prepare_class_maps(class_feature_maps, normalise=True):
    lib = _lib.load()
    if isinstance(class_feature_maps, torch.Tensor):
        class_feature_maps = [m.unsqueeze(0) for m in class_feature_maps]
    if len(class_feature_maps) == 0:
        raise RuntimeError("need at least one class feature map")
    maps = []
    for fm in class_feature_maps:
        fm = _require_device_f32(fm, "class feature map")
        if fm.dim() == 4:
            assert fm.size(0) == 1, "Can process only batches of size 1, but have {0}".format(fm.size(0))
            fm = fm[0]
        maps.append(fm)
    C = maps[0].size(0)
    dev = maps[0].device
    B = len(maps)
    for fm in maps:
        if fm.size(0) != C:
            raise RuntimeError("class feature maps disagree on the feature dimension: {} vs {}".format(fm.size(0), C))
        if fm.device != dev:
            raise RuntimeError("class feature maps are on different devices: {} vs {}".format(fm.device, dev))
    q15 = torch.empty(B, C, TEMPLATE, TEMPLATE, dtype=torch.float32, device=dev)
    qp = torch.empty(B, C, QROWS, dtype=torch.float32, device=dev)
    with torch.cuda.device(dev):
        for b0 in range(0, B, 65535):
            chunk = maps[b0:b0 + 65535]
            ptrs = torch.tensor([m.data_ptr() for m in chunk], dtype=torch.int64).to(dev, non_blocking=False)
            sizes = torch.tensor([[m.size(1), m.size(2)] for m in chunk], dtype=torch.int32).to(dev, non_blocking=False)
            ws = torch.empty(lib.os2d_class_prepare_workspace_floats(len(chunk), C), dtype=torch.float32, device=dev)
            _lib.call("os2d_class_prepare_batch", ptrs, sizes, len(chunk), C, 1 if normalise else 0, q15[b0:b0 + len(chunk)],
                      qp[b0:b0 + len(chunk)], ws, STREAM)
            cur = torch.cuda.current_stream(dev)
            ptrs.record_stream(cur), sizes.record_stream(cur), ws.record_stream(cur)
            for m in chunk:
                m.record_stream(cur)
    return q15, qp


class Os2dHead(nn.Module):

    def __init__(self, class_feature_maps, aligner, box_grid_generator_image_level,
                 box_grid_generator_feature_map_level, pool_border_width=2, _prepared=None, _stride=None,
                 _rec_field=None):
        super(Os2dHead, self).__init__()
        if pool_border_width != 2:
            raise RuntimeError("the HIP resampling kernel is built for pool_border_width=2 (the only value the "
                               "reference uses, head.py:280)")
        class_feature_maps = _require_device_f32(class_feature_maps, "class_feature_maps")
        if class_feature_maps.dim() != 4 or class_feature_maps.size(2) != TEMPLATE or class_feature_maps.size(3) != TEMPLATE:
            raise RuntimeError("class_feature_maps must be [B,C,15,15], got {}".format(tuple(class_feature_maps.shape)))
        if _prepared is None:
            class_feature_maps, _prepared = _prepare_class_maps(class_feature_maps, normalise=True)
        self.class_feature_maps = class_feature_maps
        self._raw_class_maps = None
        self._qp = _prepared
        self._qs = None
        self.class_batch_size = self.class_feature_maps.size(0)
        self.box_grid_generator_image_level = box_grid_generator_image_level
        self.box_grid_generator_feature_map_level = box_grid_generator_feature_map_level
        mask = torch.zeros(self.class_batch_size, 1, TEMPLATE, TEMPLATE, dtype=torch.float32,
                           device=self.class_feature_maps.device)
        mask[:, :, pool_border_width:TEMPLATE - pool_border_width, pool_border_width:TEMPLATE - pool_border_width] = 1
        self.class_pool_mask = mask / mask.sum(dim=(2, 3), keepdim=True)
        self.aligner = aligner
        self.last_precision = None
        self.precision = None
        self.train_precision = None
        self.last_train_precision = None
        self.train_forward_precision = None
        self.last_train_forward_precision = None
        self.keep_train_activations = False
        self.last_train_activations = None
        self.deterministic = None
        self.last_deterministic = None
        self.last_live_batchnorm = None
        self._status = None
        self.strict_range = os.environ.get("OS2D_STRICT_RANGE", "0") not in ("0", "", "false")
        box = box_grid_generator_image_level
        self._stride = int(box.box_stride.w)
        self._rec_field = int(box.box_size.w - self._stride * (TEMPLATE - 1))
        if box.box_stride.w != box.box_stride.h or box.box_size.w != box.box_size.h:
            raise RuntimeError("anisotropic strides / receptive fields are not supported by the HIP head")

    def _split_class_operand(self):
        dev = self._qp.device
        if self._qs is None:
            lib = _lib.load()
            B, C = self._qp.size(0), self._qp.size(1)
            qs = torch.empty(lib.os2d_class_split_bytes(B, C), dtype=torch.uint8, device=dev)
            _lib.call("os2d_class_split", self._qp, qs, B, C, STREAM)
            self._qs = _StreamOrdered(None, qs, dev)
        return self._qs.get(dev)

    def prepare(self, precision=None):
        precision = resolve_precision(precision or self.precision)
        self.aligner.parameter_regressor.packed(precision)
        if precision not in FP32_MODES:
            self._split_class_operand()
        return self

    def _status_word(self):
        if self._status is None:
            self._status = device_status_word(self._qp.device, owner=self)
        return self._status

    def range_status(self, synchronize=False):
        if synchronize:
            torch.cuda.synchronize(self._qp.device)
        return int(self._status_word()[0])

    def clear_range_status(self):
        self._status_word()[0] = 0

    @classmethod
    def cat(cls, heads):
        h0 = heads[0]
        q15 = torch.cat([h.class_feature_maps for h in heads], 0)
        qp = torch.cat([h._qp for h in heads], 0)
        return cls(q15, h0.aligner, h0.box_grid_generator_image_level, h0.box_grid_generator_feature_map_level,
                   _prepared=qp)

    def forward(self, feature_maps, out=None, stage_events=None, precision=None, strict_range=None, route_pairs=None):
        feature_maps = _require_device_f32(feature_maps, "feature_maps")
        if feature_maps.dim() != 4:
            raise RuntimeError("feature_maps must be [A,C,H,W], got {}".format(tuple(feature_maps.shape)))
        _resolve(precision or self.precision)
        if out is None and stage_events is None and (head_train.needs_grad(self, feature_maps)
                                                      or any(self.aligner.parameter_regressor.live_batchnorm())):
            if feature_maps.size(1) != self.class_feature_maps.size(1):
                raise RuntimeError("Feature dimensionality of input={0} and class={1} feature maps has to equal".format(
                    feature_maps.size(1), self.class_feature_maps.size(1)))
            return head_train.head_forward_train(self, feature_maps)
        if torch.is_grad_enabled() and feature_maps.requires_grad:
            raise RuntimeError("autograd through the HIP head does not take preallocated outputs or stage events: "
                               "call under torch.no_grad()")
        A, C, H, W = feature_maps.shape
        B = self.class_batch_size
        class_feature_dim = self.class_feature_maps.size(1)
        assert C == class_feature_dim, \
            "Feature dimensionality of input={0} and class={1} feature maps has to equal".format(C, class_feature_dim)
        if self._qp.device != feature_maps.device:
            raise RuntimeError("class features are on {} but feature_maps on {}".format(self._qp.device, feature_maps.device))
        dev = feature_maps.device
        regressor = self.aligner.parameter_regressor
        P = regressor.output_dim
        precision, pinned = _resolve(precision or self.precision)
        regressor.check_ready()
        spectra = None
        if W > MAX_W_DIRECT7:
            precision = {"f32": "fft32", "f16x3": "fftx3", "f16x2": "fftx3"}.get(precision, precision)
            pinned = True
        if precision in FFT_MODES:
            pairs = A * B if route_pairs is None else int(route_pairs)
            spectra = regressor.spectra(H, W, split=precision == "fftx3") if (pinned or pairs >= FFT_MIN_PAIRS) else None
            if spectra is None:
                precision = "f32" if precision == "fft32" else "f16x3"
        spectra2 = None
        if precision == "fftx3" and spectra is not None and not os.environ.get("OS2D_CONV2_FREQ", "1").startswith("0"):
            spectra2 = regressor.spectra2(H, W)
        self.last_precision = precision
        w1, b1, w2, b2, w3, b3 = regressor.packed(precision)
        if out is None:
            loc = torch.empty(A, B, 4, H, W, dtype=torch.float32, device=dev)
            cls = torch.empty(A, B, 1, H, W, dtype=torch.float32, device=dev)
            corners = torch.empty(A, B, 8, H, W, dtype=torch.float32, device=dev)
        else:
            loc, cls, corners = out
            for t, k in ((loc, 4), (cls, 1), (corners, 8)):
                if tuple(t.shape) != (A, B, k, H, W) or not t.is_contiguous() or t.device != dev or t.dtype != torch.float32:
                    raise RuntimeError("out tensors must be contiguous float32 [A,B,{},H,W] on {}".format(k, dev))
        full = ctypes.c_size_t()
        one = ctypes.c_size_t()
        _lib.call("os2d_head_workspace_bytes_ex", A, B, C, H, W, P, PRECISIONS[precision], ctypes.byref(full))
        _lib.call("os2d_head_workspace_bytes_ex", A, 1, C, H, W, P, PRECISIONS[precision], ctypes.byref(one))
        with torch.cuda.device(dev):
            ws = get_workspace(dev, min(full.value, workspace_cap_bytes()), one.value)
            status = self._status_word() if precision not in FP32_MODES else None
            _lib.call("os2d_head_forward_ex2", feature_maps, self._qp, w1, b1, w2, b2, w3, b3, A, B, C, H, W, P,
                      1 if self.aligner.use_inverse_geom_model else 0, self._stride, self._rec_field, loc, cls, corners, ws, ws.numel(),
                      STREAM, PRECISIONS[precision], self._split_class_operand() if precision not in FP32_MODES else None, stage_events,
                      None, _lib.host_ptr(status), *(spectra[:3] if spectra is not None else (None, None, None)), spectra2)
        strict = self.strict_range if strict_range is None else strict_range
        if strict and precision not in FP32_MODES:
            torch.cuda.current_stream(dev).synchronize()
            if int(self._status[0]) != 0:
                self.clear_range_status()
                logging.getLogger("OS2D").warning("OS2D head: non-finite input or an activation outside the fp16 range; strict_range "
                                                  "re-runs this call in precision='f32'")
                return self.forward(feature_maps, out=out, stage_events=stage_events, precision="f32")
        return loc, cls, cls, corners


def normalize_feature_map_L2(feature_maps, epsilon=1e-6):
    return feature_maps / (feature_maps.norm(dim=1, keepdim=True) + epsilon)
```

### os2d_amd/modeling/spectra.py

```python
import collections
import ctypes
import functools
import itertools
import os

import torch

from .. import _lib
from .._native import STREAM


@functools.lru_cache(maxsize=None)
def transform_sizes(H, W, split):
    lib = _lib.load()
    out = [ctypes.c_int() for _ in range(7)]
    ref = [ctypes.byref(x) for x in out]
    if split:
        tiles = (ctypes.c_int * 6)()
        rc = lib.os2d_dft_sizes(H, W, *ref[:3], tiles)
    else:
        rc = lib.os2d_fft_sizes(H, W, *ref[:3]) or lib.os2d_fft_tiles(H, W, *ref[3:])
        tiles = [x.value for x in out[3:]]
    return tuple(x.value for x in out[:3]) + (tuple(tiles),) if rc == 0 else None


def twiddles64(n, device):
    m = torch.arange(n, dtype=torch.float64)
    ang = m * (-2.0 * torch.pi / n)
    return torch.stack([torch.cos(ang), torch.sin(ang)], 1).to(device).contiguous()


def build_dft_matrices(P, Q, device):
    lib = _lib.load()
    tp64, tq64 = twiddles64(P, device), twiddles64(Q, device)
    mats = torch.empty(lib.os2d_dft_matrices_bytes(P, Q), dtype=torch.uint8, device=device)
    _lib.call("os2d_dft_matrices_build", tp64, tq64, P, Q, mats, STREAM)
    cur = torch.cuda.current_stream(device)
    tp64.record_stream(cur), tq64.record_stream(cur)
    return mats


def build_weight_spectra(wfold, C, Cout, P, Q, nbins, split, device):
    lib = _lib.load()
    wfold = wfold.to(device).contiguous()
    tp64, tq64 = twiddles64(P, device), twiddles64(Q, device)
    scratch = torch.empty(1024, dtype=torch.uint8, device=device)
    args = (wfold, tp64, tq64, C, Cout, P, Q, nbins)
    if split:
        wspec = torch.empty(lib.os2d_spectral_weight16_bytes(C, nbins), dtype=torch.uint8, device=device)
        _lib.call("os2d_spectral_weights_build_dft", *args, wspec, scratch, STREAM)
    else:
        wspec = torch.empty(lib.os2d_spectral_weight_bytes(C, Cout, nbins) // 4, dtype=torch.float32, device=device)
        _lib.call("os2d_spectral_weights_build", *args, 0, wspec, scratch, STREAM)
    cur = torch.cuda.current_stream(device)
    for t in (wfold, tp64, tq64, scratch):
        t.record_stream(cur)
    return wspec


class _StreamOrdered(object):

    def __init__(self, key, value, device):
        self.key, self.value = key, value
        stream = torch.cuda.current_stream(device)
        self._stream = stream.cuda_stream
        self._event = torch.cuda.Event()
        self._event.record(stream)

    def get(self, device):
        stream = torch.cuda.current_stream(device)
        if stream.cuda_stream != self._stream:
            stream.wait_event(self._event)
            for t in self._tensors():
                t.record_stream(stream)
        return self.value

    def _tensors(self):
        values = self.value if isinstance(self.value, (tuple, list)) else (self.value,)
        return [t for t in values if isinstance(t, torch.Tensor)]

    def nbytes(self):
        return sum(t.numel() * t.element_size() for t in self._tensors())


def spectra_cache_cap_bytes(split=True):
    env = os.environ.get("OS2D_FFT_CACHE_BYTES")
    if env:
        return int(env)
    total = 64 << 30
    if torch.cuda.is_available():
        total = torch.cuda.get_device_properties(torch.cuda.current_device()).total_memory
    return int(min(8 << 30, total // 8)) if split else int(min(64 << 30, total // 4))


class _SpectraStore(object):
    _stores = {}

    @classmethod
    def of(cls, device):
        index = device.index if device.index is not None else torch.cuda.current_device()
        store = cls._stores.get(index)
        if store is None:
            store = cls._stores[index] = cls()
        return store

    def __init__(self):
        self.entries = collections.OrderedDict()

    def get(self, net_id, slot, key):
        entry = self.entries.get((net_id, slot))
        if entry is None or entry.key != key:
            return None
        self.entries.move_to_end((net_id, slot))
        return entry

    def drop_stale(self, net_id, key):
        for k in [k for k, e in self.entries.items() if k[0] == net_id and e.key != key]:
            del self.entries[k]

    def drop_net(self, net_id):
        for k in [k for k in self.entries if k[0] == net_id]:
            del self.entries[k]

    def put(self, net_id, slot, entry):
        family = bool(slot[2])
        cap, used = spectra_cache_cap_bytes(family), entry.nbytes()
        for k in list(self.entries):
            if used + sum(e.nbytes() for kk, e in self.entries.items() if bool(kk[1][2]) == family) <= cap:
                break
            if bool(k[1][2]) == family:
                del self.entries[k]
        self.entries[(net_id, slot)] = entry

    def slots_of(self, net_id):
        return [k[1] for k in self.entries if k[0] == net_id]

    def nbytes(self):
        return sum(e.nbytes() for e in self.entries.values())


def split_rows_f16(T):
    dims = tuple(range(1, T.dim()))
    amax = T.abs().amax(dim=dims).clamp_min(1e-300)
    wexp = torch.floor(torch.log2(32768.0 / amax)).clamp(-100, 100)
    T *= torch.exp2(wexp).view(-1, *([1] * (T.dim() - 1)))
    hi = T.to(torch.float16)
    T -= hi.double()
    lo = T.to(torch.float16)
    return hi, lo, wexp



_NET_IDS = itertools.count(1)


class _SpectraView(object):

    def __init__(self, store, net_id):
        self.store, self.net_id = store, net_id

    def __len__(self):
        return len(self.store.slots_of(self.net_id))

    def __contains__(self, slot):
        return (self.net_id, slot) in self.store.entries

    def __iter__(self):
        return iter(self.store.slots_of(self.net_id))

    def values(self):
        return [e for k, e in self.store.entries.items() if k[0] == self.net_id]

    def clear(self):
        self.store.drop_net(self.net_id)


def _drop_spectra_of(net_id):
    for store in _SpectraStore._stores.values():
        store.drop_net(net_id)
```

Measured before the change: 51090.

## Generate conv2 weight spectra on the fly from per-row partial DFTs in spectral GEMM

Adds a compact 'rows' weight representation for the 5x5 conv2 layer. It holds each filter's column-DFT per frequency column v, folded into symmetric and antisymmetric tap sums, plus a small twiddle table. A new spectral GEMM variant rebuilds the full per-bin weight spectrum in registers from these rows, so it no longer streams a large precomputed per-bin spectrum from memory. The aim is to cut weight-spectrum memory traffic and cache footprint in exchange for extra FMA work per bin. It falls back to the streamed spectra when the pair count exceeds a kernel limit.

New measurement: 51210, median of 6. About the same (+0.2%).

```diff
diff --git a/include/os2d_hip.h b/include/os2d_hip.h
--- a/include/os2d_hip.h
+++ b/include/os2d_hip.h
@@ -64,6 +64,12 @@
                           void* workspace, size_t workspace_bytes, void* stream, int precision, const void* qs,
                           void** stage_events, int* chunk_classes, int* status, const float* wspec, const float* twQ,
                           const float* twP, const void* wspec2);
+int os2d_head_forward_ex3(const float* fm, const float* qp, const void* w1, const float* b1, const void* w2,
+                          const float* b2, const void* w3, const float* b3, int A, int B, int C, int H, int W, int P,
+                          int inverse, int stride, int rec_field, float* loc, float* cls, float* corners,
+                          void* workspace, size_t workspace_bytes, void* stream, int precision, const void* qs,
+                          void** stage_events, int* chunk_classes, int* status, const float* wspec, const float* twQ,
+                          const float* twP, const void* wspec2, const void* wrows2);
 void os2d_debug_set_dump(void* stream, int slot, void* dst, size_t bytes);
 int os2d_prof_event_create(void** ev);
 int os2d_prof_event_destroy(void* ev);
@@ -148,6 +154,12 @@
 int os2d_spectral_gemm_f16_quads(const void* w16, const float* X, float* Y, int NB, int C, int Cout, int nbins, float xscale,
                                  void* stream);
 float os2d_dft_xscale(int H, int W);
+size_t os2d_spectral_rows_bytes(int C, int P, int Q, int taps);
+int os2d_spectral_rows_build(const double* wfold, const double* twP64, const double* twQ64, int C, int Cout, int P, int Q,
+                             int taps, void* out, void* workspace, void* stream);
+int os2d_spectral_gemm_f16_rows(const void* rows, const void* w16, const float* X, float* Y, int NB, int C, int Cout, int nbins,
+                                int P, int Q, int taps, float xscale, void* stream);
+int os2d_spectral_gen_max_pairs(void);
 
 #define OS2D_PYRAMID_MAX_LEVELS 16
 int os2d_detect_pyramid_supported(int L, int N, int nms_max_batch);
diff --git a/os2d_amd/_lib.py b/os2d_amd/_lib.py
--- a/os2d_amd/_lib.py
+++ b/os2d_amd/_lib.py
@@ -56,6 +56,12 @@
                                   ctypes.POINTER(_vp), ctypes.POINTER(_i), _vp, _vp, _vp, _vp]),
     "os2d_head_forward_ex2": (_i, [_vp] * 8 + [_i] * 9 + [_vp, _vp, _vp, _vp, _sz, _vp, _i, _vp,
                                    ctypes.POINTER(_vp), ctypes.POINTER(_i), _vp, _vp, _vp, _vp, _vp]),
+    "os2d_head_forward_ex3": (_i, [_vp] * 8 + [_i] * 9 + [_vp, _vp, _vp, _vp, _sz, _vp, _i, _vp,
+                                   ctypes.POINTER(_vp), ctypes.POINTER(_i), _vp, _vp, _vp, _vp, _vp, _vp]),
+    "os2d_spectral_rows_bytes": (_sz, [_i, _i, _i, _i]),
+    "os2d_spectral_rows_build": (_i, [_vp, _vp, _vp, _i, _i, _i, _i, _i, _vp, _vp, _vp]),
+    "os2d_spectral_gemm_f16_rows": (_i, [_vp, _vp, _vp, _vp, _i, _i, _i, _i, _i, _i, _i, _f, _vp]),
+    "os2d_spectral_gen_max_pairs": (_i, []),
     "os2d_dft_inverse_planes": (_i, [_vp, _vp, _vp, _vp, _i, _i, _i, _i, _vp, _vp]),
     "os2d_head_workspace_bytes_ex": (_i, [_i, _i, _i, _i, _i, _i, _i, ctypes.POINTER(_sz)]),
     "os2d_prof_event_create": (_i, [ctypes.POINTER(_vp)]),
diff --git a/os2d_amd/csrc/abi.hip b/os2d_amd/csrc/abi.hip
--- a/os2d_amd/csrc/abi.hip
+++ b/os2d_amd/csrc/abi.hip
@@ -377,6 +377,26 @@
   return os2d_launch_spectral_gemm_f16(w16, X, Y, NB, C, Cout, nbins, xscale, 1, os2d_dft_channel_stride(C), os2d_stream(stream));
 }
 
+size_t os2d_spectral_rows_bytes(int C, int P, int Q, int taps) { return C < 1 ? 0 : os2d_spectral_rows_size(C, P, Q, taps); }
+
+int os2d_spectral_rows_build(const double* wfold, const double* twP64, const double* twQ64, int C, int Cout, int P, int Q,
+                             int taps, void* out, void* workspace, void* stream) {
+  if (!wfold || !twP64 || !twQ64 || !out || !workspace || C < 1 || Cout < 1 || Cout > 64 || !os2d_spectral_rows_size(C, P, Q, taps))
+    return OS2D_REFUSE(-1, "os2d_spectral_rows_build: bad arguments (C=%d Cout=%d P=%d Q=%d taps=%d)", C, Cout, P, Q, taps);
+  if (!aligned_to(16, out) || !aligned_to(8, workspace)) return OS2D_REFUSE(-1, "os2d_spectral_rows_build: out must be 16-byte, workspace 8-byte aligned");
+  return os2d_launch_spectra_rows(wfold, twP64, twQ64, C, Cout, P, Q, taps, out, workspace, os2d_stream(stream));
+}
+
+int os2d_spectral_gemm_f16_rows(const void* rows, const void* w16, const float* X, float* Y, int NB, int C, int Cout, int nbins,
+                                int P, int Q, int taps, float xscale, void* stream) {
+  if (!spectral_gemm_args_ok("os2d_spectral_gemm_f16_rows", "", rows, X, Y, NB, C, Cout, nbins, xscale)) return -1;
+  if (!aligned_to(16, w16)) return OS2D_REFUSE(-1, "os2d_spectral_gemm_f16_rows: buffers must be 16-byte aligned");
+  return os2d_launch_spectral_gemm_f16_rows(rows, w16, X, Y, NB, C, Cout, nbins, P, Q, taps, xscale, 1, os2d_dft_channel_stride(C),
+                                            os2d_stream(stream));
+}
+
+int os2d_spectral_gen_max_pairs(void) { return os2d_spectral_gen_max_pairs_value(); }
+
 float os2d_dft_xscale(int H, int W) {
   int t[6];
   if (H < 1 || W < 1 || !os2d_dft_plan(H, W, nullptr, nullptr, nullptr, t)) return 0.f;
diff --git a/os2d_amd/csrc/head_call.hip b/os2d_amd/csrc/head_call.hip
--- a/os2d_amd/csrc/head_call.hip
+++ b/os2d_amd/csrc/head_call.hip
@@ -20,6 +20,7 @@
   int layout;
   int bins, tiles[6], T;
   int xch;
+  int P2, Q2;
 };
 
 struct Span {
@@ -100,7 +101,7 @@
   return s;
 }
 bool precision_route(int precision, HeadRoute* r) {
-  *r = HeadRoute{precision, false, T7_NONE, false, false, false, 3, OS2D_SPECTRA_ROWS, 0, {1, 1, 0, 0, 0, 0}, 1, L1.cin};
+  *r = HeadRoute{precision, false, T7_NONE, false, false, false, 3, OS2D_SPECTRA_ROWS, 0, {1, 1, 0, 0, 0, 0}, 1, L1.cin, 0, 0};
   switch (precision) {
     case OS2D_PRECISION_F32: return true;
     case OS2D_PRECISION_F16X3: r->f16 = true; return true;
@@ -117,7 +118,7 @@
     if (launch && W > OS2D_MAX_W_DIRECT7)
       return OS2D_REFUSE(-1, "feature map width %d > %d: the direct 7x7 kernels keep 3 halo rows of their input in LDS - wider maps need a "
                          "frequency-domain precision (fftx3 / fft / fft32), which tiles any width up to %d", W, OS2D_MAX_W_DIRECT7, OS2D_MAX_W);
-  } else if (!(r->transform == T7_DFT ? os2d_dft_plan : os2d_fft_plan)(H, W, nullptr, nullptr, &r->bins, r->tiles)) {
+  } else if (!(r->transform == T7_DFT ? os2d_dft_plan : os2d_fft_plan)(H, W, &r->P2, &r->Q2, &r->bins, r->tiles)) {
     return OS2D_REFUSE(-3, "%s: no transform plan for a %dx%d map", who, H, W);
   }
   r->T = r->tiles[0] * r->tiles[1];
@@ -150,7 +151,7 @@
 
 struct HeadCall {
   const float *fm, *qp, *b1, *b2, *b3, *wspec, *twQ, *twP;
-  const void *w1, *w2, *w3, *qs, *wspec2;
+  const void *w1, *w2, *w3, *qs, *wspec2, *wrows2;
   int A, B, C, H, W, P, inverse, stride, rec_field;
   float *loc, *cls, *corners;
   int* status;
@@ -223,7 +224,8 @@
     return r.f16 ? os2d_launch_conv_f16x3(2, x.h1, x.w2, x.b2, x.whole_call, x.h2, NB, x.P, H, W, 3, x.st)
                  : os2d_launch_conv(2, x.h1, static_cast<const float*>(x.w2), x.b2, x.h2, NB, x.P, H, W, x.st);
   if ((rc = os2d_launch_dft_forward(x.h1, nullptr, x.xspec, x.twQ, NB, L2.cin, L2.cin, H, W, x.st))) return rc;
-  if ((rc = os2d_launch_spectral_gemm_f16(x.wspec2, x.xspec, x.yspec, NB * r.T, L2.cin, L2.cout, r.bins, os2d_spectral_xscale_for(r.tiles[4], r.tiles[5]), 1, L2.cin, x.st)))
+  if ((rc = os2d_launch_spectral_gemm_f16_rows(x.wrows2, x.wspec2, x.xspec, x.yspec, NB * r.T, L2.cin, L2.cout, r.bins, r.P2, r.Q2, L2.ks,
+                                               os2d_spectral_xscale_for(r.tiles[4], r.tiles[5]), 1, L2.cin, x.st)))
     return rc;
   return os2d_launch_dft_inverse(x.yspec, x.b2, L2.rows, x.h2, x.twQ, NB, L2.cout, H, W, x.whole_call, OS2D_DFT_OUT_SHB_BORDERS, x.st);
 }
@@ -275,19 +277,19 @@
   return head_workspace_bytes("os2d_head_workspace_bytes_ex", A, B, C, H, W, P, precision, bytes);
 }
 
-int os2d_head_forward_ex2(const float* fm, const float* qp, const void* w1, const float* b1, const void* w2,
+int os2d_head_forward_ex3(const float* fm, const float* qp, const void* w1, const float* b1, const void* w2,
                           const float* b2, const void* w3, const float* b3, int A, int B, int C, int H, int W, int P,
                           int inverse, int stride, int rec_field, float* loc, float* cls, float* corners,
                           void* workspace, size_t workspace_bytes, void* stream, int precision, const void* qs,
                           void** stage_events, int* chunk_classes, int* status, const float* wspec, const float* twQ,
-                          const float* twP, const void* wspec2) {
+                          const float* twP, const void* wspec2, const void* wrows2) {
   if (!fm || !qp || !w1 || !b1 || !w2 || !b2 || !w3 || !b3 || !loc || !cls || !corners || !workspace) return OS2D_REFUSE(-1, "os2d_head_forward: null pointer");
   HeadRoute route;
   precision_route(precision, &route);
   if (route.transform != T7_NONE && (!wspec || !twQ || (route.transform != T7_DFT && !twP)))
     return OS2D_REFUSE(-1, "os2d_head_forward: the frequency-domain modes need the weight spectra and the transform tables "
                        "(fft / fft32: twQ, twP; fftx3: the matrices of os2d_dft_matrices_build as twQ)");
-  int rc = head_route("os2d_head_forward", precision, H, W, wspec2 != nullptr, true, &route);
+  int rc = head_route("os2d_head_forward", precision, H, W, wspec2 != nullptr || wrows2 != nullptr, true, &route);
   if (rc) return rc;
   if (route.f16 && !qs) return OS2D_REFUSE(-1, "os2d_head_forward: precision f16x3 / f16x2 needs the split class operand (os2d_class_split)");
   if (!head_args_ok(A, B, C, H, W, P)) return -1;
@@ -298,7 +300,7 @@
     return OS2D_REFUSE(-2, "os2d_head_forward: workspace too small (%zu B, need >= %zu B for one class)", workspace_bytes,
                        carve(route, A, 1, C, H, W, P).total);
   if (chunk_classes) *chunk_classes = Bc;
-  HeadCall x = {fm, qp, b1, b2, b3, wspec, twQ, twP, w1, w2, w3, qs, wspec2, A, B, C, H, W, P, inverse, stride, rec_field, loc, cls, corners,
+  HeadCall x = {fm, qp, b1, b2, b3, wspec, twQ, twP, w1, w2, w3, qs, wspec2, wrows2, A, B, C, H, W, P, inverse, stride, rec_field, loc, cls, corners,
                 status, stage_events, os2d_stream(stream), carve(route, A, Bc, C, H, W, P)};
   const Carve& c = x.layout;
   char* ws = static_cast<char*>(workspace);
@@ -314,6 +316,10 @@
   x.xspec = route.bins ? floats(c.xspec) : nullptr;
   x.yspec = route.bins ? floats(c.yspec) : nullptr;
   x.sumfx = (route.bins && route.f16 && os2d_corr_f16x3_use_packed(A, Bc, H, W)) ? ws + c.sumfx.at : nullptr;
+  if (x.wrows2 && route.conv2_freq && (long long)A * Bc * route.T > os2d_spectral_gen_max_pairs_value()) {
+    if (!wspec2) return OS2D_REFUSE(-1, "os2d_head_forward: %d pairs per launch need the streamed weight spectra of the 5x5 layer (wspec2)", A * Bc * route.T);
+    x.wrows2 = nullptr;
+  }
   x.flags = route.f16 ? reinterpret_cast<int*>(ws + c.flags.at) : nullptr;
   x.epoch = next_epoch();
   x.per_image = {x.flags, x.epoch};
@@ -343,6 +349,16 @@
   return 0;
 }
 
+int os2d_head_forward_ex2(const float* fm, const float* qp, const void* w1, const float* b1, const void* w2,
+                          const float* b2, const void* w3, const float* b3, int A, int B, int C, int H, int W, int P,
+                          int inverse, int stride, int rec_field, float* loc, float* cls, float* corners,
+                          void* workspace, size_t workspace_bytes, void* stream, int precision, const void* qs,
+                          void** stage_events, int* chunk_classes, int* status, const float* wspec, const float* twQ,
+                          const float* twP, const void* wspec2) {
+  return os2d_head_forward_ex3(fm, qp, w1, b1, w2, b2, w3, b3, A, B, C, H, W, P, inverse, stride, rec_field, loc, cls, corners, workspace,
+                               workspace_bytes, stream, precision, qs, stage_events, chunk_classes, status, wspec, twQ, twP, wspec2, nullptr);
+}
+
 int os2d_head_forward_ex(const float* fm, const float* qp, const void* w1, const float* b1, const void* w2,
                          const float* b2, const void* w3, const float* b3, int A, int B, int C, int H, int W, int P,
                          int inverse, int stride, int rec_field, float* loc, float* cls, float* corners,
diff --git a/os2d_amd/csrc/os2d_common.h b/os2d_amd/csrc/os2d_common.h
--- a/os2d_amd/csrc/os2d_common.h
+++ b/os2d_amd/csrc/os2d_common.h
@@ -125,6 +125,8 @@
 int os2d_launch_spectra_pack(const double* wfold, const double* twP64, const double* twQ64, int C, int Cout, int P, int Q,
                              int NBINS, int split, int u_fastest ,
                              void* out, void* workspace, hipStream_t stream);
+int os2d_launch_spectra_rows(const double* wfold, const double* twP64, const double* twQ64, int C, int Cout, int P, int Q, int taps,
+                             void* out, void* workspace, hipStream_t stream);
 size_t os2d_spectral_weight_floats(int C, int Cout, int NBINS);
 int os2d_launch_spectral_gemm(const float* wspec, const float* X, float* Y, int NB, int C, int Cout, int NBINS,
                               hipStream_t stream);
@@ -133,6 +135,10 @@
 int os2d_launch_spectral_gemm_f16(const void* w16, const float* X, float* Y, int NB, int C, int Cout, int NBINS, float xscale,
                                   int x_quads , int Cpad,
                                   hipStream_t stream);
+size_t os2d_spectral_rows_size(int C, int P, int Q, int taps);
+int os2d_spectral_gen_max_pairs_value();
+int os2d_launch_spectral_gemm_f16_rows(const void* rows , const void* w16 , const float* X, float* Y, int NB, int C,
+                                       int Cout, int NBINS, int P, int Q, int taps, float xscale, int x_quads, int Cpad, hipStream_t stream);
 int os2d_dft_plan(int H, int W, int* P, int* Q, int* nbins, int* tiles );
 size_t os2d_dft_matrices_size(int P, int Q);
 int os2d_launch_dft_matrices(const double* twP64, const double* twQ64, int P, int Q, void* out, hipStream_t stream);
diff --git a/os2d_amd/csrc/spectra_pack.hip b/os2d_amd/csrc/spectra_pack.hip
--- a/os2d_amd/csrc/spectra_pack.hip
+++ b/os2d_amd/csrc/spectra_pack.hip
@@ -1,4 +1,5 @@
 #include "tile_common.h"
+#include "spectral_gen.h"
 
 namespace {
 
@@ -39,6 +40,9 @@
                                                               int C, int Cout, int P, int Q, int NBINS, int bins_per_block,
                                                               unsigned long long* __restrict__ amax, void* __restrict__ out,
                                                               float* __restrict__ wscale, int ufast) {
+  const int ufast_arg = ufast;
+  const bool rows = MODE == 1 && (ufast & 2);
+  ufast &= 1;
   extern __shared__ __attribute__((aligned(16))) unsigned char smem[];
   cd* tP = reinterpret_cast<cd*>(smem);
   cd* tQ = tP + P;
@@ -73,6 +77,44 @@
     e = max(-100, min(100, e));
     scale = ldexp(1.0, e);
     if (blockIdx.x % (KSTEPS * 2) == 0 && blockIdx.y == 0 && c4 == 0 && o < 128) wscale[o] = (float)ldexp(1.0, -e);
+  }
+  if (rows) {
+    const int T = (ufast_arg >> 4) & 7, t0 = gen_first_tap(T);
+    f32x2* G = reinterpret_cast<f32x2*>(out);
+    if (blockIdx.x == 0 && blockIdx.y == 0) {
+      cd* tw = reinterpret_cast<cd*>(G + gen_g_elems(C, V, T));
+      for (int i = tid; i < P * (T / 2); i += SP_THR) {
+        const int u = i / (T / 2), pt = (SP_R - (t0 + i % (T / 2)) + P) % P;
+        tw[i] = tP[(u * pt) % P];
+      }
+    }
+    if (half) return;
+    for (int v = bin0; v < min(bin0 + bins_per_block, V); ++v) {
+      cd eq[SP_KS];
+#pragma unroll
+      for (int s = 0; s < SP_KS; ++s) eq[s] = tQ[(v * ((SP_R - s + Q) % Q)) % Q];
+      cd g[SP_KS];
+#pragma unroll
+      for (int t = 0; t < SP_KS; ++t) {
+        g[t] = cd{0.0, 0.0};
+#pragma unroll
+        for (int s = 0; s < SP_KS; ++s) {
+          g[t].re = fma(w[t * SP_KS + s], eq[s].re, g[t].re);
+          g[t].im = fma(w[t * SP_KS + s], eq[s].im, g[t].im);
+        }
+      }
+#pragma unroll
+      for (int t = 0; t <= SP_R; ++t) {
+        if (t < t0) continue;
+        const cd a = t < SP_R ? cd{g[t].re + g[SP_KS - 1 - t].re, g[t].im + g[SP_KS - 1 - t].im} : g[t];
+        G[gen_g_index(v, c, ol, t - t0, KSTEPS, T)] = f32x2{(float)(a.re * scale), (float)(a.im * scale)};
+        if (t < SP_R) {
+          const cd d = cd{g[t].re - g[SP_KS - 1 - t].re, g[t].im - g[SP_KS - 1 - t].im};
+          G[gen_g_index(v, c, ol, SP_KS - 1 - t - t0, KSTEPS, T)] = f32x2{(float)(d.re * scale), (float)(d.im * scale)};
+        }
+      }
+    }
+    return;
   }
   for (int bin = bin0; bin < bin1; ++bin) {
     cd k{0.0, 0.0};
@@ -133,3 +175,28 @@
                      out, nullptr, u_fastest);
   return os2d_launched("spectra_pack (complex64)");
 }
+
+int os2d_launch_spectra_rows(const double* wfold, const double* twP64, const double* twQ64, int C, int Cout, int P, int Q, int taps,
+                             void* out, void* workspace, hipStream_t stream) {
+  const int V = Q / 2 + 1, KSTEPS = (C + 7) / 8, NBINS = os2d_round_up(P * V, 8);
+  if (Cout > GEN_ROWS || Q < 2 || (Q & 1) || !gen_code_ok(P, V, taps)) {
+    os2d_set_error("spectra_rows: bad sizes (P=%d Q=%d Cout=%d taps=%d)", P, Q, Cout, taps);
+    return -3;
+  }
+  const size_t lds = (size_t)(P + Q) * sizeof(cd);
+  const int nb_y = 8, per = os2d_round_up((NBINS + nb_y - 1) / nb_y, 8), perv = (V + nb_y - 1) / nb_y;
+  unsigned long long* amax = static_cast<unsigned long long*>(workspace);
+  hipError_t e = hipMemsetAsync(amax, 0, 128 * sizeof(unsigned long long), stream);
+  if (e != hipSuccess) {
+    os2d_set_error("hipMemsetAsync: %s", hipGetErrorString(e));
+    return -4;
+  }
+  hipLaunchKernelGGL(spectra_pack_kernel<0>, dim3(2 * KSTEPS * 2, (NBINS + per - 1) / per), dim3(SP_THR), lds, stream, wfold, twP64, twQ64, C,
+                     Cout, P, Q, NBINS, per, amax, nullptr, nullptr, 1);
+  int rc = os2d_launched("spectra_pack (row maxima)");
+  if (rc) return rc;
+  float* wscale = reinterpret_cast<float*>(static_cast<char*>(out) + gen_rows_size(C, P, Q, taps)) - 128;
+  hipLaunchKernelGGL(spectra_pack_kernel<1>, dim3(2 * KSTEPS * 2, (V + perv - 1) / perv), dim3(SP_THR), lds, stream, wfold, twP64, twQ64, C,
+                     Cout, P, Q, NBINS, perv, amax, out, wscale, 1 | 2 | (taps << 4));
+  return os2d_launched("spectra_pack (rows)");
+}
diff --git a/os2d_amd/csrc/spectral_f16.hip b/os2d_amd/csrc/spectral_f16.hip
--- a/os2d_amd/csrc/spectral_f16.hip
+++ b/os2d_amd/csrc/spectral_f16.hip
@@ -1,4 +1,6 @@
 #include "tile_common.h"
+#include "spectral_gen.h"
+#include <type_traits>
 
 namespace {
 
@@ -10,21 +12,30 @@
 constexpr int SH_KC = 8;
 constexpr int SH_STAGE = SH_WB * 2 * 2 * 64;
 constexpr int SH_WSTAGE = 2 * SH_STAGE;
+constexpr int SH_GEN_MAX_PAIRS = 0;
 constexpr int SH_WRING = 2;
 
 #define SH_MM(x_, y_, acc_) __builtin_amdgcn_mfma_f32_32x32x16_f16(x_, y_, acc_, 0, 0, 0)
 __device__ __forceinline__ void sh_lds_barrier() { asm volatile("s_waitcnt lgkmcnt(0)\n\ts_barrier" ::: "memory"); }
 
-template <bool XQ, bool R64>
+__device__ __forceinline__ void sh_quad_exchange(unsigned (&x)[4]) {
+  u32x2 a = __builtin_amdgcn_permlane16_swap(x[0], x[1], false, false), b = __builtin_amdgcn_permlane16_swap(x[2], x[3], false, false);
+  const u32x2 c = __builtin_amdgcn_permlane32_swap(a[0], b[0], false, false), d = __builtin_amdgcn_permlane32_swap(a[1], b[1], false, false);
+  x[0] = c[0], x[2] = c[1], x[1] = d[0], x[3] = d[1];
+}
+
+template <bool XQ, bool R64, int GT = 0>
 __device__ __forceinline__ void spectral_gemm_f16_body(const u32x4* w16,
                                                        const float* __restrict__ wscale,
                                                        const f32x2* __restrict__ X,
                                                        f32x2* __restrict__ Y,
-                                                       int NB, int C, int Cpad, int Cout, int NBINS, float xscale, int nunits) {
+                                                       int NB, int C, int Cpad, int Cout, int NBINS, float xscale, int nunits, int gen = 0) {
+  static_assert(GT == 0 || R64, "the generator lives in the 64-row shape");
+  constexpr bool GEN = GT > 0;
   extern __shared__ __attribute__((aligned(16))) unsigned char smem[];
   constexpr int JB = R64 ? SH_WB / 2 : SH_WB;
   constexpr int WSTAGE = R64 ? SH_STAGE : SH_WSTAGE;
-  constexpr int NWL = WSTAGE / SH_THR, NXL = SH_STAGE / SH_THR;
+  constexpr int NWL = GEN ? GT : WSTAGE / SH_THR, NXL = SH_STAGE / SH_THR;
   u32x4* ldsW = reinterpret_cast<u32x4*>(smem);
   u32x4* ldsX = ldsW + SH_WRING * WSTAGE;
   const int tid = threadIdx.x, lane = tid & 63, l31 = lane & 31, hw = lane >> 5;
@@ -53,17 +64,54 @@
   const u32x4* wbase = w16 + ((size_t)(g * 2 + (R64 ? 0 : wh)) * KS) * (SH_BINS * 256) + bh * SH_STAGE;
 #define SH_WRUN(K) (R64 ? wv * 2 + (K) : wq * 4 + (K))
 #define SH_WPART (R64 ? 0 : wh * SH_STAGE)
-  u32x4 wra[NWL], wrb[NWL];
+  std::conditional_t<GEN, f32x2, u32x4> wra[NWL], wrb[NWL];
+  constexpr int GP = GEN ? GT / 2 : 1, GTT = GEN ? GT : 1;
+  const int gq = wv & 1, go = (wv >> 1) * 16 + (lane & 15), gch = lane >> 4;
+  const int gP = gen_code_P(gen), gV = gen_code_V(gen);
+  const int gv = GEN ? bin0 / gP : 0, gu0 = GEN ? bin0 - gv * gP : 0;
+  const bool gpad = GEN && gv >= gV;
+  const f32x2* gbase = reinterpret_cast<const f32x2*>(w16) + ((size_t)min(gv, gV - 1) * KS * 2 + gq) * (GTT * 256) + go * 4 + gch;
+  const size_t gks = 2 * GTT * 256;
+#ifndef OS2D_GEN_REAL
+#define OS2D_GEN_REAL double
+#endif
+  typedef OS2D_GEN_REAL gen_real;
+  typedef gen_real gen_real2 __attribute__((ext_vector_type(2)));
+  gen_real2 gtw[4][GP];
+  if constexpr (GEN) {
+    const f64x2* tw_ = reinterpret_cast<const f64x2*>(wscale);
+#pragma unroll
+    for (int b = 0; b < 4; ++b)
+#pragma unroll
+      for (int k = 0; k < GP; ++k) gtw[b][k] = __builtin_convertvector(tw_[(gu0 + b) * GP + k], gen_real2);
+    wscale += 2 * gen_tw_elems(gP, GT);
+  }
 #define SH_LOAD_W(S, wr)                                                                                            \
   {                                                                                                                 \
-    const u32x4* src_ = wbase + (size_t)(S) * (SH_BINS * 256);                                                      \
-    _Pragma("unroll") for (int k_ = 0; k_ < NWL; ++k_) wr[k_] = src_[SH_WRUN(k_) * 64 + lane];                      \
+    if constexpr (GEN) {                                                                                            \
+      _Pragma("unroll") for (int k_ = 0; k_ < NWL; ++k_) wr[k_] = gbase[(size_t)(S) * gks + k_ * 256];              \
+    } else {                                                                                                        \
+      const u32x4* src_ = wbase + (size_t)(S) * (SH_BINS * 256);                                                    \
+      _Pragma("unroll") for (int k_ = 0; k_ < NWL; ++k_) wr[k_] = src_[SH_WRUN(k_) * 64 + lane];                    \
+    }                                                                                                               \
   }
 #define SH_LOAD_W1(S, wr, K) wr[K] = (wbase + (size_t)(S) * (SH_BINS * 256))[SH_WRUN(K) * 64 + lane];
 #define SH_STORE_W(S, wr)                                                                                           \
   {                                                                                                                 \
-    _Pragma("unroll") for (int k_ = 0; k_ < NWL; ++k_)                                                              \
-        ldsW[((S) % SH_WRING) * WSTAGE + SH_WPART + SH_WRUN(k_) * 64 + lane] = wr[k_];                             \
+    if constexpr (GEN) {                                                                                            \
+      gen_real gr_[4], gi_[4];                                                                                       \
+      unsigned gh_[4], gl_[4];                                                                                      \
+      gen_values<GTT>(wr, gtw, gr_, gi_);                                                                           \
+      _Pragma("unroll") for (int b_ = 0; b_ < 4; ++b_) gen_split(gpad ? (gen_real)0 : gr_[b_], gpad ? (gen_real)0 : gi_[b_], &gh_[b_], &gl_[b_]); \
+      sh_quad_exchange(gh_);                                                                                        \
+      sh_quad_exchange(gl_);                                                                                        \
+      u32x4* dst_ = ldsW + ((S) % SH_WRING) * WSTAGE + ((gch * 2 + gq) * 2) * 64 + go;                              \
+      dst_[0] = u32x4{gh_[0], gh_[1], gh_[2], gh_[3]};                                                              \
+      dst_[64] = u32x4{gl_[0], gl_[1], gl_[2], gl_[3]};                                                             \
+    } else {                                                                                                        \
+      _Pragma("unroll") for (int k_ = 0; k_ < NWL; ++k_)                                                            \
+          ldsW[((S) % SH_WRING) * WSTAGE + SH_WPART + SH_WRUN(k_) * 64 + lane] = wr[k_];                           \
+    }                                                                                                               \
   }
   const int xn = XQ ? wv * 8 + (lane >> 3) : wq * 16 + (lane & 15);
   const int xj = XQ ? (lane & 1) : (lane >> 4) & 1, xg = XQ ? (lane >> 2) & 1 : lane >> 5;
@@ -120,7 +168,16 @@
     __builtin_amdgcn_sched_barrier(0);                                                                              \
   }
 #define SH_REQUESTS_HOOK(SN, WN, PN, J)                                                                             \
-  if ((J) == 0) {                                                                                                   \
+  if constexpr (GEN) {                           \
+    if ((J) == 0) {                                                                                                 \
+      SH_LOAD_W(SN, WN)                                                                                             \
+      __builtin_amdgcn_sched_barrier(0);                                                                            \
+    } else if ((J) == 1) {                                                                                          \
+      SH_LOAD_X1(SN, PN, 0)                                                                                         \
+      SH_LOAD_X1(SN, PN, 1)                                                                                         \
+      __builtin_amdgcn_sched_barrier(0);                                                                            \
+    }                                                                                                               \
+  } else if ((J) == 0) {                                                                                            \
     SH_REQUEST2(SN, WN, PN, 0)                                                                                      \
   } else if ((J) == 1) {                                                                                            \
     SH_REQUEST2(SN, WN, PN, 2)                                                                                      \
@@ -231,7 +288,11 @@
                                                                       const f32x2* __restrict__ X, f32x2* __restrict__ Y, int NB, int C,
                                                                       int Cpad, int Cout, int NBINS, int rows64, float xscale,
                                                                       int nunits) {
-  if (rows64)
+  if (gen_code_taps(rows64) == 5)
+    spectral_gemm_f16_body<XQ, true, 5>(w16, wscale, X, Y, NB, C, Cpad, Cout, NBINS, xscale, nunits, rows64);
+  else if (gen_code_taps(rows64) == 7)
+    spectral_gemm_f16_body<XQ, true, 7>(w16, wscale, X, Y, NB, C, Cpad, Cout, NBINS, xscale, nunits, rows64);
+  else if (rows64)
     spectral_gemm_f16_body<XQ, true>(w16, wscale, X, Y, NB, C, Cpad, Cout, NBINS, xscale, nunits);
   else
     spectral_gemm_f16_body<XQ, false>(w16, wscale, X, Y, NB, C, Cpad, Cout, NBINS, xscale, nunits);
@@ -250,8 +311,22 @@
   return s;
 }
 
-int os2d_launch_spectral_gemm_f16(const void* w16, const float* X, float* Y, int NB, int C, int Cout, int NBINS, float xscale,
-                                  int x_quads, int Cpad, hipStream_t stream) {
+size_t os2d_spectral_rows_size(int C, int P, int Q, int taps) {
+  return (Q >= 2 && !(Q & 1) && gen_code_ok(P, Q / 2 + 1, taps)) ? gen_rows_size(C, P, Q, taps) : 0;
+}
+
+int os2d_spectral_gen_max_pairs_value() {
+  static const int v = [] {
+    const char* e = getenv("OS2D_GEMM_GEN");
+    if (!e || !e[0]) return SH_GEN_MAX_PAIRS;
+    const long n = strtol(e, nullptr, 10);
+    return n <= 0 ? 0 : n == 1 ? 0x7fffffff : (int)(n < 0x7fffffffL ? n : 0x7fffffffL);
+  }();
+  return v;
+}
+
+int os2d_launch_spectral_gemm_f16_rows(const void* rows, const void* w16, const float* X, float* Y, int NB, int C, int Cout, int NBINS,
+                                       int P, int Q, int taps, float xscale, int x_quads, int Cpad, hipStream_t stream) {
   if (NBINS % SH_BINS || Cout > 2 * SH_OH) {
     os2d_set_error("spectral_gemm_f16: NBINS %d must be a multiple of %d and Cout %d <= %d", NBINS, SH_BINS, Cout, 2 * SH_OH);
     return -3;
@@ -265,16 +340,38 @@
     return !(e && e[0] == '0');
   }();
   const bool r64 = Cout <= SH_OH && rows64_env;
+  static const bool gen_env = [] {
+    const char* e = getenv("OS2D_GEMM_GEN");
+    return !(e && e[0] == '0');
+  }();
+  const int V = Q / 2 + 1;
+  const bool gen = rows && r64 && gen_env && (NB <= os2d_spectral_gen_max_pairs_value() || !w16);
+  if (gen && (!gen_code_ok(P, V, taps) || (Q & 1) || P * V > NBINS || NBINS - P * V >= SH_BINS)) {
+    os2d_set_error("spectral_gemm_f16: rows operand of P=%d Q=%d taps=%d does not fit %d bins", P, Q, taps, NBINS);
+    return -3;
+  }
+  if (!gen && !w16) {
+    os2d_set_error("spectral_gemm_f16: no streamed weight spectra, and the generated path does not apply (Cout %d, %d pairs)", Cout, NB);
+    return -1;
+  }
   const int G = NBINS / SH_BINS, nbt = (NB + SH_NB - 1) / SH_NB;
   const size_t KS = (size_t)(C + SH_KC - 1) / SH_KC;
-  const float* wscale = reinterpret_cast<const float*>(static_cast<const char*>(w16) + (size_t)G * 2 * KS * SH_BINS * 256 * 16);
+  const void* wop = gen ? rows : w16;
+  const float* wscale = gen ? reinterpret_cast<const float*>(rows) + 2 * gen_g_elems(C, V, taps)
+                            : reinterpret_cast<const float*>(static_cast<const char*>(w16) + (size_t)G * 2 * KS * SH_BINS * 256 * 16);
   const size_t lds = (size_t)(SH_WRING * (r64 ? SH_STAGE : SH_WSTAGE) + 2 * SH_STAGE) * 16;
   const long long units = (long long)G * nbt * (SH_BINS / SH_WB);
   unsigned grid;
   if (int rc = os2d_xcd_grid(units, "spectral_gemm_f16", &grid)) return rc;
   auto kern = x_quads ? spectral_gemm_f16_kernel<true> : spectral_gemm_f16_kernel<false>;
   if (int rc = os2d_set_dynamic_lds(kern, lds, "spectral_gemm_f16")) return rc;
-  hipLaunchKernelGGL(kern, dim3(grid), dim3(SH_THR), lds, stream, static_cast<const u32x4*>(w16), wscale,
-                     reinterpret_cast<const f32x2*>(X), reinterpret_cast<f32x2*>(Y), NB, C, Cpad, Cout, NBINS, (int)r64, xscale, (int)units);
+  hipLaunchKernelGGL(kern, dim3(grid), dim3(SH_THR), lds, stream, static_cast<const u32x4*>(wop), wscale,
+                     reinterpret_cast<const f32x2*>(X), reinterpret_cast<f32x2*>(Y), NB, C, Cpad, Cout, NBINS,
+                     gen ? gen_code(P, V, taps) : (int)r64, xscale, (int)units);
   return os2d_launched("spectral_gemm_f16");
 }
+
+int os2d_launch_spectral_gemm_f16(const void* w16, const float* X, float* Y, int NB, int C, int Cout, int NBINS, float xscale,
+                                  int x_quads, int Cpad, hipStream_t stream) {
+  return os2d_launch_spectral_gemm_f16_rows(nullptr, w16, X, Y, NB, C, Cout, NBINS, 0, 0, 0, xscale, x_quads, Cpad, stream);
+}
diff --git a/os2d_amd/csrc/spectral_gen.h b/os2d_amd/csrc/spectral_gen.h
--- /dev/null
+++ b/os2d_amd/csrc/spectral_gen.h
@@ -0,0 +1,72 @@
+#pragma once
+#include "tile_common.h"
+#include <stddef.h>
+
+#ifdef OS2D_HOST_EMU
+#define GEN_DEV static inline
+#define GEN_HD static inline
+#else
+#define GEN_DEV __device__ __forceinline__
+#define GEN_HD static inline __host__ __device__
+#endif
+
+constexpr int GEN_MAX_TAPS = 7;
+constexpr int GEN_ROWS = 64;
+
+GEN_HD bool gen_taps_ok(int T) { return T == 5 || T == 7; }
+GEN_HD int gen_first_tap(int T) { return (GEN_MAX_TAPS - T) / 2; }
+GEN_HD size_t gen_kstep_elems(int T) { return (size_t)2 * T * GEN_ROWS * 4; }
+GEN_HD size_t gen_g_elems(int C, int V, int T) { return (size_t)V * ((C + 7) / 8) * gen_kstep_elems(T); }
+GEN_HD size_t gen_tw_elems(int P, int T) { return (size_t)P * (T / 2) * 2; }
+GEN_HD size_t gen_rows_size(int C, int P, int Q, int T) {
+  return (gen_g_elems(C, Q / 2 + 1, T) + gen_tw_elems(P, T)) * 2 * sizeof(float) + 128 * sizeof(float);
+}
+GEN_HD size_t gen_g_index(int v, int c, int o, int k, int KS, int T) {
+  return ((((size_t)v * KS + (c >> 3)) * 2 + ((c >> 2) & 1)) * T + k) * (GEN_ROWS * 4) + (size_t)o * 4 + (c & 3);
+}
+
+GEN_HD bool gen_code_ok(int P, int V, int T) { return gen_taps_ok(T) && P >= 4 && P < 1024 && (P & 3) == 0 && V >= 1 && V < (1 << 17); }
+GEN_HD int gen_code(int P, int V, int T) { return 1 | (T << 1) | (P << 4) | (V << 14); }
+GEN_HD int gen_code_taps(int code) { return (code >> 1) & 7; }
+GEN_HD int gen_code_P(int code) { return (code >> 4) & 1023; }
+GEN_HD int gen_code_V(int code) { return (code >> 14) & 0x1ffff; }
+
+typedef double f64x2 __attribute__((ext_vector_type(2)));
+GEN_DEV double gen_fma(double a, double b, double c) { return __builtin_fma(a, b, c); }
+GEN_DEV float gen_fma(float a, float b, float c) { return __builtin_fmaf(a, b, c); }
+
+template <int T, class R, class E2>
+GEN_DEV void gen_values(const f32x2 (&g)[T], const E2 (&e)[4][T / 2], R (&wr)[4], R (&wi)[4]) {
+#pragma unroll
+  for (int b = 0; b < 4; ++b) {
+    wr[b] = (R)g[T / 2][0];
+    wi[b] = (R)g[T / 2][1];
+  }
+#pragma unroll
+  for (int k = 0; k < T / 2; ++k) {
+    const R sx = (R)g[k][0], sy = (R)g[k][1], dx = (R)g[T - 1 - k][0], dy = (R)g[T - 1 - k][1];
+#pragma unroll
+    for (int b = 0; b < 4; ++b) {
+      const R c = e[b][k][0], s = e[b][k][1];
+      wr[b] = gen_fma(sx, c, wr[b]);
+      wr[b] = gen_fma(-dy, s, wr[b]);
+      wi[b] = gen_fma(sy, c, wi[b]);
+      wi[b] = gen_fma(dx, s, wi[b]);
+    }
+  }
+}
+
+GEN_DEV void gen_split(double re, double im, unsigned* hi, unsigned* lo) {
+  const _Float16 hr = (_Float16)(float)re, hi_ = (_Float16)(float)im;
+  const _Float16 lr = (_Float16)(float)(re - (double)hr), li = (_Float16)(float)(im - (double)hi_);
+  *hi = (unsigned)__builtin_bit_cast(unsigned short, hr) | ((unsigned)__builtin_bit_cast(unsigned short, hi_) << 16);
+  *lo = (unsigned)__builtin_bit_cast(unsigned short, lr) | ((unsigned)__builtin_bit_cast(unsigned short, li) << 16);
+}
+#ifndef OS2D_HOST_EMU
+GEN_DEV void gen_split(float re, float im, unsigned* hi, unsigned* lo) {
+  typedef _Float16 half2_ __attribute__((ext_vector_type(2)));
+  const f32x2 v = {re, im};
+  *hi = __builtin_bit_cast(unsigned, __builtin_convertvector(v, half2_));
+  *lo = os2d_split_lo_pair(re, im, *hi);
+}
+#endif
diff --git a/os2d_amd/modeling/head.py b/os2d_amd/modeling/head.py
--- a/os2d_amd/modeling/head.py
+++ b/os2d_amd/modeling/head.py
@@ -15,7 +15,7 @@
 from .device_buffers import (STATUS_SLOTS, _WORKSPACES, device_status_word, get_workspace, release_workspaces,
                              workspace_cap_bytes)
 from .spectra import (_NET_IDS, _SpectraStore, _SpectraView, _StreamOrdered, _drop_spectra_of, build_dft_matrices,
-                      build_weight_spectra, spectra_cache_cap_bytes, split_rows_f16, transform_sizes, twiddles64)
+                      build_weight_rows, build_weight_spectra, spectra_cache_cap_bytes, split_rows_f16, transform_sizes, twiddles64)
 
 TEMPLATE = 15
 QROWS = 256
@@ -324,11 +324,18 @@
 
     def spectra2(self, H, W):
         def build(P, Q, nbins, dev):
-            _, (w2, _), _ = self._folded()
-            unit_exp = self._f16x3_plan()["unit_exp"].to(w2.device).double()
-            w2 = nn.functional.pad(w2 * torch.exp2(-unit_exp).view(1, -1, 1, 1), (1, 1, 1, 1))
-            return build_weight_spectra(w2, 128, 64, P, Q, nbins, True, dev)
+            return build_weight_spectra(self._conv2_filters7(), 128, 64, P, Q, nbins, True, dev)
         return self._cached_spectra(H, W, True, ("conv2",), build)
+
+    def _conv2_filters7(self):
+        _, (w2, _), _ = self._folded()
+        unit_exp = self._f16x3_plan()["unit_exp"].to(w2.device).double()
+        return nn.functional.pad(w2 * torch.exp2(-unit_exp).view(1, -1, 1, 1), (1, 1, 1, 1))
+
+    def spectra2_rows(self, H, W):
+        def build(P, Q, nbins, dev):
+            return build_weight_rows(self._conv2_filters7(), 128, 64, P, Q, 5, dev)
+        return self._cached_spectra(H, W, True, ("conv2rows",), build)
 
     @property
     def _spectra_cache(self):
@@ -613,9 +620,13 @@
             spectra = regressor.spectra(H, W, split=precision == "fftx3") if (pinned or pairs >= FFT_MIN_PAIRS) else None
             if spectra is None:
                 precision = "f32" if precision == "fft32" else "f16x3"
-        spectra2 = None
+        spectra2 = rows2 = None
         if precision == "fftx3" and spectra is not None and not os.environ.get("OS2D_CONV2_FREQ", "1").startswith("0"):
-            spectra2 = regressor.spectra2(H, W)
+            gen_pairs = _lib.load().os2d_spectral_gen_max_pairs()
+            tiles = transform_sizes(H, W, True)[3]
+            rows2 = regressor.spectra2_rows(H, W) if gen_pairs > 0 else None
+            if rows2 is None or A * B * tiles[0] * tiles[1] > gen_pairs:
+                spectra2 = regressor.spectra2(H, W)
         self.last_precision = precision
         w1, b1, w2, b2, w3, b3 = regressor.packed(precision)
         if out is None:
@@ -634,10 +645,10 @@
         with torch.cuda.device(dev):
             ws = get_workspace(dev, min(full.value, workspace_cap_bytes()), one.value)
             status = self._status_word() if precision not in FP32_MODES else None
-            _lib.call("os2d_head_forward_ex2", feature_maps, self._qp, w1, b1, w2, b2, w3, b3, A, B, C, H, W, P,
+            _lib.call("os2d_head_forward_ex3", feature_maps, self._qp, w1, b1, w2, b2, w3, b3, A, B, C, H, W, P,
                       1 if self.aligner.use_inverse_geom_model else 0, self._stride, self._rec_field, loc, cls, corners, ws, ws.numel(),
                       STREAM, PRECISIONS[precision], self._split_class_operand() if precision not in FP32_MODES else None, stage_events,
-                      None, _lib.host_ptr(status), *(spectra[:3] if spectra is not None else (None, None, None)), spectra2)
+                      None, _lib.host_ptr(status), *(spectra[:3] if spectra is not None else (None, None, None)), spectra2, rows2)
         strict = self.strict_range if strict_range is None else strict_range
         if strict and precision not in FP32_MODES:
             torch.cuda.current_stream(dev).synchronize()
diff --git a/os2d_amd/modeling/spectra.py b/os2d_amd/modeling/spectra.py
--- a/os2d_amd/modeling/spectra.py
+++ b/os2d_amd/modeling/spectra.py
@@ -56,6 +56,22 @@
     for t in (wfold, tp64, tq64, scratch):
         t.record_stream(cur)
     return wspec
+
+
+def build_weight_rows(wfold, C, Cout, P, Q, taps, device):
+    lib = _lib.load()
+    nbytes = lib.os2d_spectral_rows_bytes(C, P, Q, taps)
+    if not nbytes:
+        return None
+    wfold = wfold.to(device).contiguous()
+    tp64, tq64 = twiddles64(P, device), twiddles64(Q, device)
+    scratch = torch.empty(1024, dtype=torch.uint8, device=device)
+    rows = torch.empty(nbytes, dtype=torch.uint8, device=device)
+    _lib.call("os2d_spectral_rows_build", wfold, tp64, tq64, C, Cout, P, Q, taps, rows, scratch, STREAM)
+    cur = torch.cuda.current_stream(device)
+    for t in (wfold, tp64, tq64, scratch):
+        t.record_stream(cur)
+    return rows
 
 
 class _StreamOrdered(object):
```
